# microsoft/ptgnn

Hardware: NVIDIA H100
Metric: edges/sec per GNN layer (higher is better)
Workload: dtype f32

## Files before the change

### include/ptgnn_b200.h

```cpp
#ifndef PTGNN_B200_H_
#define PTGNN_B200_H_

#include <stddef.h>
#include <stdint.h>

#ifdef __cplusplus
extern "C" {
#endif

#define PTGNN_B200_ABI_VERSION 4
#define PTGNN_MAX_EDGE_TYPES 128

enum {
    PTGNN_OK = 0,
    PTGNN_E_INVALID = -1,
    PTGNN_E_UNSUPPORTED = -2,
    PTGNN_E_CUDA = -3,
    PTGNN_E_WORKSPACE = -4,
    PTGNN_E_INDEX = -5
};

enum { PTGNN_REDUCE_SUM = 0, PTGNN_REDUCE_MEAN = 1, PTGNN_REDUCE_MAX = 2, PTGNN_REDUCE_MIN = 3 };
enum { PTGNN_ACT_NONE = 0, PTGNN_ACT_GELU = 1, PTGNN_ACT_TANH = 2, PTGNN_ACT_RELU = 3 };

int ptgnn_b200_abi_version(void);
const char *ptgnn_b200_last_error(void);
int64_t ptgnn_b200_launch_count(void);

enum {
    PTGNN_KERNEL_PLAN = 0,
    PTGNN_KERNEL_MESSAGE = 1,
    PTGNN_KERNEL_REDUCE = 2,
    PTGNN_KERNEL_GRU = 3,
    PTGNN_KERNEL_DENSE = 4,
    PTGNN_KERNEL_PACK = 5,
    PTGNN_KERNEL_CATEGORIES = 6
};
int ptgnn_b200_kernel_timing_enable(int32_t enable);
int ptgnn_b200_kernel_timing_read(double *ms , int64_t *launches , int32_t ncat);

size_t ptgnn_b200_plan_workspace_bytes(int64_t num_nodes, int64_t num_edges);
int ptgnn_b200_plan_build(int64_t num_nodes, int64_t num_source_nodes ,
                          int32_t num_types,
                          const int64_t *const *src_ptrs ,
                          const int64_t *const *tgt_ptrs ,
                          const int64_t *counts , int32_t *row_ptr, int32_t *perm,
                          int32_t *pos, int32_t *src_sorted, uint8_t *etype_sorted, int32_t *src32, int32_t *tgt32,
                          int32_t *status, void *workspace, size_t workspace_bytes, void *stream);

int ptgnn_b200_plan_convert(int64_t num_nodes, int64_t num_source_nodes, int32_t num_types,
                            const int64_t *const *src_ptrs , const int64_t *const *tgt_ptrs ,
                            const int64_t *counts , int32_t *row_ptr, int32_t *src32, int32_t *tgt32, int32_t *status,
                            void *workspace, size_t workspace_bytes, void *stream);
int ptgnn_b200_plan_sort(int64_t num_nodes, int32_t num_types, const int64_t *counts , int32_t *perm, int32_t *pos,
                         int32_t *src_sorted, uint8_t *etype_sorted, const int32_t *src32, const int32_t *tgt32,
                         void *workspace, size_t workspace_bytes, void *stream);

int ptgnn_b200_segment_reduce_f32(const float *messages, const int32_t *row_ptr, const int32_t *perm,
                                  int64_t num_nodes, int64_t num_edges, int32_t dim, int32_t reduce, float *out,
                                  int64_t *arg_out, void *stream);

size_t ptgnn_b200_scatter_workspace_bytes(int64_t num_nodes, int64_t num_edges);
int ptgnn_b200_scatter_f32(const float *src, const int64_t *index, int64_t num_edges, int32_t dim, int64_t num_nodes,
                           int32_t reduce, float *out, int64_t *arg_out, int32_t *status, void *workspace,
                           size_t workspace_bytes, void *stream);

size_t ptgnn_b200_gated_workspace_bytes(int32_t bf16_states, int64_t num_nodes, int64_t num_edges, int32_t num_types,
                                        int32_t state_dim, int32_t message_dim);
size_t ptgnn_b200_gated_weight_cache_bytes(int32_t bf16_states, int32_t num_types, int32_t state_dim, int32_t message_dim);
int ptgnn_b200_gated_forward(int32_t bf16_states, const void *node_states, const void *gather_states ,
                             int64_t num_nodes, int32_t state_dim, int32_t message_dim, int32_t num_types,
                             const int64_t *type_off , const int32_t *row_ptr, const int32_t *pos, const int32_t *src32,
                             const float *const *edge_weights , const float *gru_w_ih, const float *gru_w_hh,
                             const float *gru_b_ih, const float *gru_b_hh, int32_t reduce, void *out_states, void *workspace,
                             size_t workspace_bytes, void *weight_cache, size_t weight_cache_bytes, int32_t cache_valid,
                             void *stream);

size_t ptgnn_b200_mlp_workspace_bytes(int32_t bf16_states, int64_t num_nodes, int64_t num_edges, int32_t num_types, int32_t in_dim,
                                      int32_t message_dim, int32_t out_dim, int32_t use_target_state);
int ptgnn_b200_mlp_forward(int32_t bf16_states, const void *node_states, const void *gather_states ,
                           int64_t num_nodes, int32_t in_dim, int32_t message_dim, int32_t out_dim, int32_t num_types,
                           const int64_t *type_off , const int32_t *row_ptr, const int32_t *pos, const int32_t *src32,
                           const int32_t *tgt32, const float *const *edge_weights ,
                           int32_t use_target_state, int32_t reduce, int32_t message_activation, const float *ln_weight,
                           const float *ln_bias, float ln_eps, const float *dense_weight, const float *dense_bias,
                           int32_t dense_activation, void *out_states, void *workspace, size_t workspace_bytes, void *stream);

typedef struct {
    int32_t block_targets;
    const int32_t *group_off;
    const int32_t *src_f;
    const uint8_t *tl_f;
    int32_t *status;
} ptgnn_b200_block_plan;

int32_t ptgnn_b200_block_plan_block_targets(int64_t num_nodes);
size_t ptgnn_b200_block_plan_workspace_bytes(int64_t num_nodes, int64_t num_edges, int32_t num_types, int32_t block_targets);
int ptgnn_b200_block_plan_build(int64_t num_nodes, int32_t num_types, const int64_t *type_off ,
                                const int32_t *src32, const int32_t *tgt32, int32_t block_targets, int32_t *group_off,
                                int32_t *src_f, uint8_t *tl_f, void *workspace, size_t workspace_bytes, void *stream);

int32_t ptgnn_b200_fused_supported(int32_t bf16_states, int32_t state_dim, int32_t message_dim);

size_t ptgnn_b200_gated_fused_workspace_bytes(int32_t bf16_states, int64_t num_nodes, int64_t num_source_nodes,
                                              int32_t num_types, int32_t state_dim, int32_t message_dim);
size_t ptgnn_b200_gated_fused_weight_cache_bytes(int32_t bf16_states, int32_t num_types, int32_t state_dim, int32_t message_dim);
size_t ptgnn_b200_packed_state_bytes(int64_t num_nodes, int32_t state_dim);
int ptgnn_b200_gated_forward_fused(int32_t bf16_states, const void *node_states, const void *gather_states ,
                                   const void *packed_states_in , int64_t num_nodes,
                                   int64_t num_source_nodes, int32_t state_dim, int32_t message_dim, int32_t num_types,
                                   const ptgnn_b200_block_plan *block_plan, const int32_t *row_ptr,
                                   const float *const *edge_weights , const float *gru_w_ih,
                                   const float *gru_w_hh, const float *gru_b_ih, const float *gru_b_hh, int32_t reduce,
                                   void *out_states, void *packed_states_out , void *workspace,
                                   size_t workspace_bytes, void *weight_cache, size_t weight_cache_bytes, int32_t cache_valid,
                                   void *stream);

size_t ptgnn_b200_mlp_fused_workspace_bytes(int32_t bf16_states, int64_t num_nodes, int64_t num_source_nodes, int32_t num_types,
                                            int32_t in_dim, int32_t message_dim, int32_t out_dim, int32_t use_target_state);
size_t ptgnn_b200_mlp_fused_weight_cache_bytes(int32_t bf16_states, int32_t num_types, int32_t in_dim, int32_t message_dim, int32_t out_dim,
                                               int32_t use_target_state);
int ptgnn_b200_mlp_forward_fused(int32_t bf16_states, const void *node_states, const void *gather_states ,
                                 int64_t num_nodes, int64_t num_source_nodes, int32_t in_dim, int32_t message_dim,
                                 int32_t out_dim, int32_t num_types, const ptgnn_b200_block_plan *block_plan,
                                 const int32_t *row_ptr, const float *const *edge_weights ,
                                 int32_t use_target_state, int32_t reduce, int32_t message_activation, const float *ln_weight,
                                 const float *ln_bias, float ln_eps, const float *dense_weight, const float *dense_bias,
                                 int32_t dense_activation, void *out_states, void *workspace, size_t workspace_bytes,
                                 void *weight_cache, size_t weight_cache_bytes, int32_t cache_valid, void *stream);

int ptgnn_b200_gather_split_f16(const float *x, const int32_t *index, int64_t rows_out, int32_t cols, const float *scale, void *hi,
                                void *lo, void *stream);
int ptgnn_b200_gru_gate_grads_f32(const float *gi, const float *gh, const float *h, const float *grad_out, int64_t num_nodes,
                                  int32_t state_dim, float *d_gi, float *d_gh, float *d_h_direct, void *stream);

int ptgnn_b200_offset_ids(const int32_t *local_ids, int64_t num_items, const int64_t *item_ptr, const int64_t *node_ptr,
                          int32_t num_graphs, int64_t *out, void *stream);
int ptgnn_b200_segment_ids(const int64_t *item_ptr, int32_t num_segments, int64_t num_items, int64_t *out, void *stream);

size_t ptgnn_b200_linear_workspace_bytes(int32_t in_dim, int32_t out_dim);
int ptgnn_b200_linear_f32(const float *x, int64_t rows, int32_t in_dim, const float *weight ,
                          const float *bias , int32_t out_dim, int32_t activation, float *out, void *workspace,
                          size_t workspace_bytes, void *stream);
size_t ptgnn_b200_grucell_workspace_bytes(int32_t state_dim, int32_t input_dim);
int ptgnn_b200_grucell_f32(const float *input, const float *hidden, int64_t rows, int32_t state_dim, int32_t input_dim,
                           const float *w_ih, const float *w_hh, const float *b_ih, const float *b_hh, float *out, void *workspace,
                           size_t workspace_bytes, void *stream);
size_t ptgnn_b200_edge_messages_workspace_bytes(int32_t num_types, int32_t in_dim, int32_t message_dim, int32_t use_target_state);
int ptgnn_b200_edge_messages_f32(const float *source_states, const float *target_states ,
                                 int32_t in_dim, int32_t message_dim, int32_t num_types, const int64_t *type_off ,
                                 const int32_t *src32, const int32_t *tgt32, const int32_t *out_row,
                                 const float *const *edge_weights , int32_t use_target_state,
                                 float *messages, void *workspace, size_t workspace_bytes, void *stream);

enum { PTGNN_READOUT_SUM = 0, PTGNN_READOUT_MEAN = 1, PTGNN_READOUT_WEIGHTED_SUM = 2 };
size_t ptgnn_b200_graph_readout_workspace_bytes(int64_t num_nodes, int64_t num_graphs, int32_t state_dim);
int ptgnn_b200_graph_readout(int32_t bf16_states, const void *node_states, int64_t num_nodes, int32_t state_dim, const int32_t *row_ptr,
                             const int32_t *perm, int64_t num_graphs, const float *gate_weight ,
                             int32_t mode, float *g, float *s , void *workspace, size_t workspace_bytes, void *stream);
int32_t ptgnn_b200_global_gru_supported(int32_t bf16_states, int32_t state_dim);
size_t ptgnn_b200_global_gru_workspace_bytes(int32_t bf16_states, int64_t num_nodes, int64_t num_graphs, int32_t state_dim,
                                             int32_t summary_dim);
size_t ptgnn_b200_global_gru_weight_cache_bytes(int32_t bf16_states, int32_t state_dim);
int ptgnn_b200_global_gru_update(int32_t bf16_states, const void *node_states, const void *packed_states_in, int64_t num_nodes,
                                 int32_t state_dim, const int32_t *graph_of_node, int64_t num_graphs, const float *g, int32_t summary_dim,
                                 const float *gru_w_ih, const float *gru_w_hh, const float *gru_b_ih, const float *gru_b_hh,
                                 void *out_states, void *packed_states_out, int32_t *status, void *workspace, size_t workspace_bytes,
                                 void *weight_cache, size_t weight_cache_bytes, int32_t cache_valid, void *stream);

int32_t ptgnn_b200_attention_readout_supported(int32_t bf16_states, int32_t state_dim, int32_t num_heads);
size_t ptgnn_b200_attention_readout_workspace_bytes(int64_t num_nodes, int64_t num_graphs, int32_t state_dim, int32_t num_heads);
int ptgnn_b200_attention_readout(int32_t bf16_states, const void *node_states, int64_t num_nodes, int32_t state_dim, int32_t num_heads,
                                 const int32_t *row_ptr, const int32_t *perm, int64_t num_graphs, const float *qt, float *o, float *lse,
                                 void *workspace, size_t workspace_bytes, void *stream);
int ptgnn_b200_attention_readout_backward_f32(const float *node_states, int64_t num_nodes, int32_t state_dim, int32_t num_heads,
                                              const int32_t *row_ptr, const int32_t *perm, int64_t num_graphs, const float *qt,
                                              const float *o, const float *lse, const float *d_o, float *d_x, float *d_qt,
                                              void *workspace, size_t workspace_bytes, void *stream);

int32_t ptgnn_b200_selfatt_supported(int32_t bf16_states, int32_t key_query_dim, int32_t value_dim);
size_t ptgnn_b200_selfatt_workspace_bytes(int64_t rows, int64_t num_graphs, int32_t num_heads);
int ptgnn_b200_selfatt_forward(int32_t bf16_states, const void *qkv, int64_t rows, int32_t num_heads, int32_t key_query_dim,
                               int32_t value_dim, const int32_t *row_ptr, int64_t num_graphs, int64_t max_chunk, void *o, float *lse,
                               int32_t *status, void *workspace, size_t workspace_bytes, void *stream);
int ptgnn_b200_selfatt_backward_f32(const float *qkv, int64_t rows, int32_t num_heads, int32_t key_query_dim, int32_t value_dim,
                                    const int32_t *row_ptr, int64_t num_graphs, int64_t max_chunk, const float *o, const float *lse,
                                    const float *d_o, float *d_qkv, void *workspace, size_t workspace_bytes, void *stream);

int32_t ptgnn_b200_graph_norm_supported(int32_t state_dim);
size_t ptgnn_b200_graph_norm_workspace_bytes(int64_t num_nodes, int64_t num_graphs, int32_t state_dim);
int ptgnn_b200_graph_norm_forward(int32_t bf16_states, const void *node_states, int64_t num_nodes, int32_t state_dim, const int32_t *row_ptr,
                                  const int32_t *perm, const int32_t *graph_of_node, int64_t num_graphs, const float *gamma,
                                  const float *alpha, const float *bias, float eps, void *out, float *mean, float *rstd, void *workspace,
                                  size_t workspace_bytes, void *stream);
int ptgnn_b200_graph_norm_backward_f32(const float *node_states, const float *d_out, int64_t num_nodes, int32_t state_dim,
                                       const int32_t *row_ptr, const int32_t *perm, const int32_t *graph_of_node, int64_t num_graphs,
                                       const float *gamma, const float *alpha, float eps, const float *mean, const float *rstd, float *d_x,
                                       float *d_gamma, float *d_alpha, float *d_bias, void *workspace, size_t workspace_bytes, void *stream);

int ptgnn_b200_gated_gnn_forward_host_f32(const float *node_states, int64_t num_nodes, int32_t state_dim,
                                          int32_t num_types, const int64_t *const *src_ptrs,
                                          const int64_t *const *tgt_ptrs, const int64_t *counts, int32_t num_layers,
                                          const float *const *edge_weights ,
                                          const float *const *gru_w_ih, const float *const *gru_w_hh,
                                          const float *const *gru_b_ih, const float *const *gru_b_hh,
                                          int32_t reduce, float *out_states);

#ifdef __cplusplus
}
#endif
#endif
```

### ptgnn_b200/_native.py

```python
import ctypes
import os
from typing import Optional, Sequence

import torch

_HERE = os.path.dirname(os.path.abspath(__file__))
LIB_PATH = os.path.join(_HERE, "libptgnn_b200.so")

REDUCE = {"sum": 0, "add": 0, "mean": 1, "max": 2, "min": 3}
READOUT_SUM, READOUT_MEAN, READOUT_WEIGHTED_SUM = 0, 1, 2
ACT_NONE, ACT_GELU, ACT_TANH, ACT_RELU = 0, 1, 2, 3

c_i32, c_i64, c_f32, c_void_p, c_size_t = ctypes.c_int32, ctypes.c_int64, ctypes.c_float, ctypes.c_void_p, ctypes.c_size_t

SIGNATURES = {
    "ptgnn_b200_abi_version": (ctypes.c_int, []),
    "ptgnn_b200_last_error": (ctypes.c_char_p, []),
    "ptgnn_b200_launch_count": (c_i64, []),
    "ptgnn_b200_kernel_timing_enable": (ctypes.c_int, [c_i32]),
    "ptgnn_b200_kernel_timing_read": (ctypes.c_int, [c_void_p, c_void_p, c_i32]),
    "ptgnn_b200_plan_workspace_bytes": (c_size_t, [c_i64, c_i64]),
    "ptgnn_b200_plan_build": (ctypes.c_int, [c_i64, c_i64, c_i32, c_void_p, c_void_p, c_void_p] + [c_void_p] * 8 + [c_void_p, c_size_t, c_void_p]),
    "ptgnn_b200_plan_convert": (ctypes.c_int, [c_i64, c_i64, c_i32, c_void_p, c_void_p, c_void_p, c_void_p, c_void_p, c_void_p, c_void_p, c_void_p, c_size_t, c_void_p]),
    "ptgnn_b200_plan_sort": (ctypes.c_int, [c_i64, c_i32, c_void_p, c_void_p, c_void_p, c_void_p, c_void_p, c_void_p, c_void_p, c_void_p, c_size_t, c_void_p]),
    "ptgnn_b200_segment_reduce_f32": (ctypes.c_int, [c_void_p, c_void_p, c_void_p, c_i64, c_i64, c_i32, c_i32, c_void_p, c_void_p, c_void_p]),
    "ptgnn_b200_scatter_workspace_bytes": (c_size_t, [c_i64, c_i64]),
    "ptgnn_b200_scatter_f32": (ctypes.c_int, [c_void_p, c_void_p, c_i64, c_i32, c_i64, c_i32, c_void_p, c_void_p, c_void_p, c_void_p, c_size_t, c_void_p]),
    "ptgnn_b200_gated_workspace_bytes": (c_size_t, [c_i32, c_i64, c_i64, c_i32, c_i32, c_i32]),
    "ptgnn_b200_gated_weight_cache_bytes": (c_size_t, [c_i32, c_i32, c_i32, c_i32]),
    "ptgnn_b200_gated_forward": (ctypes.c_int, [c_i32, c_void_p, c_void_p, c_i64, c_i32, c_i32, c_i32, c_void_p, c_void_p, c_void_p, c_void_p,
                                                c_void_p, c_void_p, c_void_p, c_void_p, c_void_p, c_i32, c_void_p, c_void_p, c_size_t,
                                                c_void_p, c_size_t, c_i32, c_void_p]),
    "ptgnn_b200_mlp_workspace_bytes": (c_size_t, [c_i32, c_i64, c_i64, c_i32, c_i32, c_i32, c_i32, c_i32]),
    "ptgnn_b200_mlp_forward": (ctypes.c_int, [c_i32, c_void_p, c_void_p, c_i64, c_i32, c_i32, c_i32, c_i32, c_void_p, c_void_p, c_void_p, c_void_p,
                                              c_void_p, c_void_p, c_i32, c_i32, c_i32, c_void_p, c_void_p, c_f32, c_void_p, c_void_p, c_i32,
                                              c_void_p, c_void_p, c_size_t, c_void_p]),
    "ptgnn_b200_block_plan_block_targets": (c_i32, [c_i64]),
    "ptgnn_b200_block_plan_workspace_bytes": (c_size_t, [c_i64, c_i64, c_i32, c_i32]),
    "ptgnn_b200_block_plan_build": (ctypes.c_int, [c_i64, c_i32, c_void_p, c_void_p, c_void_p, c_i32, c_void_p, c_void_p, c_void_p, c_void_p, c_size_t, c_void_p]),
    "ptgnn_b200_fused_supported": (c_i32, [c_i32, c_i32, c_i32]),
    "ptgnn_b200_gated_fused_workspace_bytes": (c_size_t, [c_i32, c_i64, c_i64, c_i32, c_i32, c_i32]),
    "ptgnn_b200_gated_fused_weight_cache_bytes": (c_size_t, [c_i32, c_i32, c_i32, c_i32]),
    "ptgnn_b200_packed_state_bytes": (c_size_t, [c_i64, c_i32]),
    "ptgnn_b200_gated_forward_fused": (ctypes.c_int, [c_i32, c_void_p, c_void_p, c_void_p, c_i64, c_i64, c_i32, c_i32, c_i32, c_void_p, c_void_p,
                                                      c_void_p, c_void_p, c_void_p, c_void_p, c_void_p, c_i32, c_void_p, c_void_p, c_void_p,
                                                      c_size_t, c_void_p, c_size_t, c_i32, c_void_p]),
    "ptgnn_b200_mlp_fused_workspace_bytes": (c_size_t, [c_i32, c_i64, c_i64, c_i32, c_i32, c_i32, c_i32, c_i32]),
    "ptgnn_b200_mlp_fused_weight_cache_bytes": (c_size_t, [c_i32, c_i32, c_i32, c_i32, c_i32, c_i32]),
    "ptgnn_b200_mlp_forward_fused": (ctypes.c_int, [c_i32, c_void_p, c_void_p, c_i64, c_i64, c_i32, c_i32, c_i32, c_i32, c_void_p, c_void_p, c_void_p,
                                                    c_i32, c_i32, c_i32, c_void_p, c_void_p, c_f32, c_void_p, c_void_p, c_i32, c_void_p, c_void_p,
                                                    c_size_t, c_void_p, c_size_t, c_i32, c_void_p]),
    "ptgnn_b200_gather_split_f16": (ctypes.c_int, [c_void_p, c_void_p, c_i64, c_i32, c_void_p, c_void_p, c_void_p, c_void_p]),
    "ptgnn_b200_gru_gate_grads_f32": (ctypes.c_int, [c_void_p, c_void_p, c_void_p, c_void_p, c_i64, c_i32, c_void_p, c_void_p, c_void_p, c_void_p]),
    "ptgnn_b200_offset_ids": (ctypes.c_int, [c_void_p, c_i64, c_void_p, c_void_p, c_i32, c_void_p, c_void_p]),
    "ptgnn_b200_segment_ids": (ctypes.c_int, [c_void_p, c_i32, c_i64, c_void_p, c_void_p]),
    "ptgnn_b200_linear_workspace_bytes": (c_size_t, [c_i32, c_i32]),
    "ptgnn_b200_linear_f32": (ctypes.c_int, [c_void_p, c_i64, c_i32, c_void_p, c_void_p, c_i32, c_i32, c_void_p, c_void_p, c_size_t, c_void_p]),
    "ptgnn_b200_grucell_workspace_bytes": (c_size_t, [c_i32, c_i32]),
    "ptgnn_b200_grucell_f32": (ctypes.c_int, [c_void_p, c_void_p, c_i64, c_i32, c_i32, c_void_p, c_void_p, c_void_p, c_void_p, c_void_p, c_void_p, c_size_t, c_void_p]),
    "ptgnn_b200_edge_messages_workspace_bytes": (c_size_t, [c_i32, c_i32, c_i32, c_i32]),
    "ptgnn_b200_edge_messages_f32": (ctypes.c_int, [c_void_p, c_void_p, c_i32, c_i32, c_i32, c_void_p, c_void_p, c_void_p, c_void_p, c_void_p,
                                                    c_i32, c_void_p, c_void_p, c_size_t, c_void_p]),
    "ptgnn_b200_graph_readout_workspace_bytes": (c_size_t, [c_i64, c_i64, c_i32]),
    "ptgnn_b200_graph_readout": (ctypes.c_int, [c_i32, c_void_p, c_i64, c_i32, c_void_p, c_void_p, c_i64, c_void_p, c_i32, c_void_p, c_void_p,
                                                c_void_p, c_size_t, c_void_p]),
    "ptgnn_b200_global_gru_supported": (c_i32, [c_i32, c_i32]),
    "ptgnn_b200_global_gru_workspace_bytes": (c_size_t, [c_i32, c_i64, c_i64, c_i32, c_i32]),
    "ptgnn_b200_global_gru_weight_cache_bytes": (c_size_t, [c_i32, c_i32]),
    "ptgnn_b200_global_gru_update": (ctypes.c_int, [c_i32, c_void_p, c_void_p, c_i64, c_i32, c_void_p, c_i64, c_void_p, c_i32, c_void_p, c_void_p,
                                                    c_void_p, c_void_p, c_void_p, c_void_p, c_void_p, c_void_p, c_size_t, c_void_p, c_size_t,
                                                    c_i32, c_void_p]),
    "ptgnn_b200_attention_readout_supported": (c_i32, [c_i32, c_i32, c_i32]),
    "ptgnn_b200_attention_readout_workspace_bytes": (c_size_t, [c_i64, c_i64, c_i32, c_i32]),
    "ptgnn_b200_attention_readout": (ctypes.c_int, [c_i32, c_void_p, c_i64, c_i32, c_i32, c_void_p, c_void_p, c_i64, c_void_p, c_void_p,
                                                    c_void_p, c_void_p, c_size_t, c_void_p]),
    "ptgnn_b200_attention_readout_backward_f32": (ctypes.c_int, [c_void_p, c_i64, c_i32, c_i32, c_void_p, c_void_p, c_i64, c_void_p, c_void_p,
                                                                 c_void_p, c_void_p, c_void_p, c_void_p, c_void_p, c_size_t, c_void_p]),
    "ptgnn_b200_selfatt_supported": (c_i32, [c_i32, c_i32, c_i32]),
    "ptgnn_b200_selfatt_workspace_bytes": (c_size_t, [c_i64, c_i64, c_i32]),
    "ptgnn_b200_selfatt_forward": (ctypes.c_int, [c_i32, c_void_p, c_i64, c_i32, c_i32, c_i32, c_void_p, c_i64, c_i64, c_void_p, c_void_p,
                                                  c_void_p, c_void_p, c_size_t, c_void_p]),
    "ptgnn_b200_selfatt_backward_f32": (ctypes.c_int, [c_void_p, c_i64, c_i32, c_i32, c_i32, c_void_p, c_i64, c_i64, c_void_p, c_void_p,
                                                       c_void_p, c_void_p, c_void_p, c_size_t, c_void_p]),
    "ptgnn_b200_graph_norm_supported": (c_i32, [c_i32]),
    "ptgnn_b200_graph_norm_workspace_bytes": (c_size_t, [c_i64, c_i64, c_i32]),
    "ptgnn_b200_graph_norm_forward": (ctypes.c_int, [c_i32, c_void_p, c_i64, c_i32, c_void_p, c_void_p, c_void_p, c_i64, c_void_p, c_void_p,
                                                     c_void_p, c_f32, c_void_p, c_void_p, c_void_p, c_void_p, c_size_t, c_void_p]),
    "ptgnn_b200_graph_norm_backward_f32": (ctypes.c_int, [c_void_p, c_void_p, c_i64, c_i32, c_void_p, c_void_p, c_void_p, c_i64, c_void_p,
                                                          c_void_p, c_f32, c_void_p, c_void_p, c_void_p, c_void_p, c_void_p, c_void_p,
                                                          c_void_p, c_size_t, c_void_p]),
    "ptgnn_b200_gated_gnn_forward_host_f32":(ctypes.c_int, [c_void_p, c_i64, c_i32, c_i32, c_void_p, c_void_p, c_void_p, c_i32,
                                                             c_void_p, c_void_p, c_void_p, c_void_p, c_void_p, c_i32, c_void_p]),
}



class BlockPlanStruct(ctypes.Structure):
    _fields_ = [("block_targets", c_i32), ("group_off", c_void_p), ("src_f", c_void_p), ("tl_f", c_void_p), ("status", c_void_p)]


ABI_VERSION = 4
_lib: Optional[ctypes.CDLL] = None


class NativeLibraryError(RuntimeError):
    pass


def lib() -> ctypes.CDLL:
    global _lib
    if _lib is None:
        if not os.path.exists(LIB_PATH):
            raise NativeLibraryError(
                f"{LIB_PATH} not found: build it with `python -m ptgnn_b200.build` (or __graft_entry__.build()). "
                "ptgnn_b200 has no CPU / PyTorch fallback for its CUDA kernels."
            )
        handle = ctypes.CDLL(LIB_PATH)
        for name, (res, args) in SIGNATURES.items():
            fn = getattr(handle, name)
            fn.restype = res
            fn.argtypes = args
        if handle.ptgnn_b200_abi_version() != ABI_VERSION:
            raise NativeLibraryError("libptgnn_b200.so ABI version mismatch; rebuild")
        _lib = handle
    return _lib


def check(rc: int, what: str) -> None:
    if rc != 0:
        msg = lib().ptgnn_b200_last_error().decode("utf-8", "replace")
        codes = {-1: ValueError, -2: NotImplementedError, -3: RuntimeError, -4: RuntimeError, -5: IndexError}
        raise codes.get(rc, RuntimeError)(f"{what} failed (code {rc}): {msg}")


def launch_count() -> int:
    return int(lib().ptgnn_b200_launch_count())


KERNEL_CATEGORIES = ("plan", "message", "reduce", "gru", "dense", "pack")


def kernel_timing(enable: bool) -> None:
    check(lib().ptgnn_b200_kernel_timing_enable(int(enable)), "kernel_timing_enable")


def read_kernel_timing() -> dict:
    n = len(KERNEL_CATEGORIES)
    ms = (ctypes.c_double * n)()
    cnt = (c_i64 * n)()
    check(lib().ptgnn_b200_kernel_timing_read(ms, cnt, n), "kernel_timing_read")
    return {name: (float(ms[i]), int(cnt[i])) for i, name in enumerate(KERNEL_CATEGORIES)}


def ptr(t: Optional[torch.Tensor]) -> Optional[int]:
    return None if t is None else t.data_ptr()


def ptr_table(tensors: Sequence[torch.Tensor]):
    tab = (c_void_p * max(len(tensors), 1))()
    for i, t in enumerate(tensors):
        tab[i] = t.data_ptr()
    return tab


def i64_array(values: Sequence[int]):
    arr = (c_i64 * max(len(values), 1))()
    for i, v in enumerate(values):
        arr[i] = int(v)
    return arr


def current_stream(device: torch.device) -> int:
    return torch.cuda.current_stream(device).cuda_stream


def require_cuda(t: torch.Tensor, name: str, dtype: torch.dtype) -> torch.Tensor:
    if not t.is_cuda:
        raise NativeLibraryError(
            f"{name} is on {t.device}; ptgnn_b200 only runs on CUDA (sm_90a) and has no CPU fallback"
        )
    if t.dtype != dtype:
        raise TypeError(f"{name} must be {dtype}, got {t.dtype}")
    return t if t.is_contiguous() else t.contiguous()
```

### ptgnn_b200/csrc/plan.cu

```cuda
#include "common.cuh"

namespace ptgnn {

constexpr int SCAN_THREADS = 256;
constexpr int SCAN_ITEMS = 16;
constexpr int SCAN_CHUNK = SCAN_THREADS * SCAN_ITEMS;

__device__ __forceinline__ int warp_inclusive_scan(int v) {
    const int lane = threadIdx.x & 31;
#pragma unroll
    for (int o = 1; o < 32; o <<= 1) {
        int n = __shfl_up_sync(0xffffffffu, v, o);
        if (lane >= o) v += n;
    }
    return v;
}

template <int THREADS>
__device__ __forceinline__ int block_exclusive_scan(int v, int *total) {
    __shared__ int warp_sums[THREADS / 32];
    __shared__ int block_total;
    const int lane = threadIdx.x & 31, warp = threadIdx.x >> 5;
    int incl = warp_inclusive_scan(v);
    if (lane == 31) warp_sums[warp] = incl;
    __syncthreads();
    if (warp == 0) {
        int s = lane < THREADS / 32 ? warp_sums[lane] : 0;
        int si = warp_inclusive_scan(s);
        if (lane < THREADS / 32) warp_sums[lane] = si - s;
        if (lane == THREADS / 32 - 1) block_total = si;
    }
    __syncthreads();
    int res = incl - v + warp_sums[warp];
    *total = block_total;
    __syncthreads();
    return res;
}

__global__ void __launch_bounds__(SCAN_THREADS) scan_block_sums_kernel(const int32_t *__restrict__ in, int64_t n,
                                                                       int32_t *__restrict__ sums) {
    const int64_t base = (int64_t)blockIdx.x * SCAN_CHUNK + (int64_t)threadIdx.x * SCAN_ITEMS;
    int s = 0;
#pragma unroll
    for (int i = 0; i < SCAN_ITEMS; ++i)
        if (base + i < n) s += in[base + i];
    int total;
    block_exclusive_scan<SCAN_THREADS>(s, &total);
    if (threadIdx.x == 0) sums[blockIdx.x] = total;
}

__global__ void __launch_bounds__(1024) scan_sums_kernel(int32_t *__restrict__ sums, int64_t nb) {
    int carry = 0;
    for (int64_t base = 0; base < nb; base += 1024) {
        int64_t i = base + threadIdx.x;
        int v = i < nb ? sums[i] : 0;
        int total;
        int ex = block_exclusive_scan<1024>(v, &total);
        if (i < nb) sums[i] = ex + carry;
        carry += total;
    }
}

__global__ void __launch_bounds__(SCAN_THREADS) scan_apply_kernel(const int32_t *in , int64_t n,
                                                                  const int32_t *__restrict__ sums, int32_t *out,
                                                                  int32_t *out_total) {
    const int64_t base = (int64_t)blockIdx.x * SCAN_CHUNK + (int64_t)threadIdx.x * SCAN_ITEMS;
    int v[SCAN_ITEMS];
    int s = 0;
#pragma unroll
    for (int i = 0; i < SCAN_ITEMS; ++i) {
        v[i] = base + i < n ? in[base + i] : 0;
        s += v[i];
    }
    int total;
    int ex = block_exclusive_scan<SCAN_THREADS>(s, &total) + sums[blockIdx.x];
#pragma unroll
    for (int i = 0; i < SCAN_ITEMS; ++i) {
        if (base + i < n) out[base + i] = ex;
        ex += v[i];
    }
    if (out_total != nullptr && blockIdx.x == gridDim.x - 1 && threadIdx.x == SCAN_THREADS - 1) out_total[0] = ex;
}

static size_t scan_workspace_elems(int64_t n) { return (size_t)ceil_div(n > 0 ? n : 1, SCAN_CHUNK) + 1; }

static int exclusive_scan_i32(const int32_t *in, int32_t *out, int64_t n, int32_t *sums, int32_t *out_total,
                              cudaStream_t st) {
    if (n <= 0) return PTGNN_OK;
    const int64_t nb = ceil_div(n, SCAN_CHUNK);
    {
        TimedScope timed__(PTGNN_KERNEL_PLAN, st);
        scan_block_sums_kernel<<<(unsigned)nb, SCAN_THREADS, 0, st>>>(in, n, sums);
    }
    PTGNN_LAUNCHED();
    {
        TimedScope timed__(PTGNN_KERNEL_PLAN, st);
        scan_sums_kernel<<<1, 1024, 0, st>>>(sums, nb);
    }
    PTGNN_LAUNCHED();
    {
        TimedScope timed__(PTGNN_KERNEL_PLAN, st);
        scan_apply_kernel<<<(unsigned)nb, SCAN_THREADS, 0, st>>>(in, n, sums, out, out_total);
    }
    PTGNN_LAUNCHED();
    return PTGNN_OK;
}

__global__ void __launch_bounds__(256) convert_count_kernel(const __grid_constant__ EdgeTables tabs, int64_t num_nodes,
                                                            int64_t num_source_nodes, int64_t num_edges, int32_t *__restrict__ src32,
                                                            int32_t *__restrict__ tgt32, int32_t *__restrict__ deg,
                                                            int32_t *__restrict__ status) {
    int bad = 0;
    for (int64_t e = (int64_t)blockIdx.x * blockDim.x + threadIdx.x; e < num_edges;
         e += (int64_t)gridDim.x * blockDim.x) {
        const int t = type_of_edge(tabs.off, tabs.num_types, e);
        const int64_t i = e - tabs.off[t];
        int64_t s = tabs.src[t][i], v = tabs.tgt[t][i];
        if (s < 0 || s >= num_source_nodes) { s = 0; ++bad; }
        if (v < 0 || v >= num_nodes) { v = 0; ++bad; }
        src32[e] = (int32_t)s;
        tgt32[e] = (int32_t)v;
        atomicAdd(&deg[v], 1);
    }
    if (bad) atomicAdd(status, bad);
}

constexpr int RADIX_BITS = 8;
constexpr int RADIX = 1 << RADIX_BITS;
constexpr int SORT_THREADS = 256;
constexpr int SORT_WARPS = SORT_THREADS / 32;
constexpr int SORT_ROUNDS = 8;
constexpr int SORT_CHUNK = SORT_THREADS * SORT_ROUNDS;

__global__ void __launch_bounds__(SORT_THREADS) radix_hist_kernel(const int32_t *__restrict__ keys, int64_t n, int shift,
                                                                  int32_t *__restrict__ hist ) {
    __shared__ int h[RADIX];
    h[threadIdx.x] = 0;
    __syncthreads();
    const int64_t base = (int64_t)blockIdx.x * SORT_CHUNK;
#pragma unroll
    for (int r = 0; r < SORT_ROUNDS; ++r) {
        int64_t i = base + r * SORT_THREADS + threadIdx.x;
        if (i < n) atomicAdd(&h[(keys[i] >> shift) & (RADIX - 1)], 1);
    }
    __syncthreads();
    hist[(int64_t)threadIdx.x * gridDim.x + blockIdx.x] = h[threadIdx.x];
}

__global__ void __launch_bounds__(SORT_THREADS) radix_scatter_kernel(const int32_t *__restrict__ keys_in,
                                                                     const int32_t *__restrict__ vals_in, int64_t n,
                                                                     int shift, int first_pass,
                                                                     const int32_t *__restrict__ hist_scanned,
                                                                     int32_t *__restrict__ keys_out,
                                                                     int32_t *__restrict__ vals_out) {
    __shared__ int warp_hist[SORT_WARPS][RADIX];
    const int lane = threadIdx.x & 31, warp = threadIdx.x >> 5;
    for (int i = threadIdx.x; i < SORT_WARPS * RADIX; i += SORT_THREADS) (&warp_hist[0][0])[i] = 0;
    __syncthreads();

    const int64_t base = (int64_t)blockIdx.x * SORT_CHUNK + warp * (32 * SORT_ROUNDS);
    int32_t key[SORT_ROUNDS], val[SORT_ROUNDS];
    int digit[SORT_ROUNDS];
#pragma unroll
    for (int r = 0; r < SORT_ROUNDS; ++r) {
        const int64_t i = base + r * 32 + lane;
        const bool valid = i < n;
        key[r] = valid ? keys_in[i] : 0;
        val[r] = valid ? (first_pass ? (int32_t)i : vals_in[i]) : 0;
        digit[r] = valid ? ((key[r] >> shift) & (RADIX - 1)) : RADIX;
        const unsigned peers = __match_any_sync(0xffffffffu, digit[r]);
        if (valid && lane == __ffs(peers) - 1) warp_hist[warp][digit[r]] += __popc(peers);
        __syncwarp();
    }
    __syncthreads();
    {
        int run = hist_scanned[(int64_t)threadIdx.x * gridDim.x + blockIdx.x];
#pragma unroll
        for (int w = 0; w < SORT_WARPS; ++w) {
            int c = warp_hist[w][threadIdx.x];
            warp_hist[w][threadIdx.x] = run;
            run += c;
        }
    }
    __syncthreads();
#pragma unroll
    for (int r = 0; r < SORT_ROUNDS; ++r) {
        const bool valid = digit[r] < RADIX;
        const unsigned peers = __match_any_sync(0xffffffffu, digit[r]);
        int dst = 0;
        if (valid) dst = warp_hist[warp][digit[r]] + __popc(peers & ((1u << lane) - 1u));
        __syncwarp();
        if (valid && lane == __ffs(peers) - 1) warp_hist[warp][digit[r]] += __popc(peers);
        __syncwarp();
        if (valid) {
            keys_out[dst] = key[r];
            vals_out[dst] = val[r];
        }
    }
}

__global__ void __launch_bounds__(256) finalize_plan_kernel(const __grid_constant__ TypeOffsets toff, int64_t num_edges,
                                                            const int32_t *__restrict__ perm,
                                                            const int32_t *__restrict__ src32,
                                                            int32_t *__restrict__ pos, int32_t *__restrict__ src_sorted,
                                                            uint8_t *__restrict__ etype_sorted) {
    for (int64_t j = (int64_t)blockIdx.x * blockDim.x + threadIdx.x; j < num_edges;
         j += (int64_t)gridDim.x * blockDim.x) {
        const int32_t e = perm[j];
        pos[e] = (int32_t)j;
        src_sorted[j] = src32[e];
        etype_sorted[j] = (uint8_t)type_of_edge(toff.off, toff.num_types, e);
    }
}

struct PlanWs {
    size_t deg, scan_sums, keys_a, keys_b, vals_a, vals_b, hist, hist_sums, total;
};
static PlanWs plan_ws_layout(int64_t N, int64_t E) {
    PlanWs w{};
    const int64_t nblk = ceil_div(E > 0 ? E : 1, SORT_CHUNK);
    size_t o = 0;
    auto add = [&](size_t cnt) { size_t at = o; o += ws_slice(cnt, 4); return at; };
    w.deg = add((size_t)N + 1);
    w.scan_sums = add(scan_workspace_elems(N + 1));
    w.keys_a = add((size_t)E + 1);
    w.keys_b = add((size_t)E + 1);
    w.vals_a = add((size_t)E + 1);
    w.vals_b = add((size_t)E + 1);
    w.hist = add((size_t)RADIX * nblk);
    w.hist_sums = add(scan_workspace_elems((int64_t)RADIX * nblk));
    w.total = o;
    return w;
}

static int sort_edges_by_key(const int32_t *keys_in, int key_bits, int64_t E, int32_t *perm, char *ws, const PlanWs &L,
                             cudaStream_t st, const int32_t **sorted_keys = nullptr) {
    const int64_t nblk = ceil_div(E, SORT_CHUNK);
    int32_t *keys[2] = {reinterpret_cast<int32_t *>(ws + L.keys_a), reinterpret_cast<int32_t *>(ws + L.keys_b)};
    int32_t *vals[2] = {reinterpret_cast<int32_t *>(ws + L.vals_a), reinterpret_cast<int32_t *>(ws + L.vals_b)};
    int32_t *hist = reinterpret_cast<int32_t *>(ws + L.hist);
    int32_t *hist_sums = reinterpret_cast<int32_t *>(ws + L.hist_sums);
    const int passes = (key_bits + RADIX_BITS - 1) / RADIX_BITS;
    const int32_t *kin = keys_in;
    const int32_t *vin = nullptr;
    for (int p = 0; p < passes; ++p) {
        int32_t *kout = keys[p & 1];
        int32_t *vout = (p == passes - 1) ? perm : vals[p & 1];
        {
            TimedScope timed__(PTGNN_KERNEL_PLAN, st);
            radix_hist_kernel<<<(unsigned)nblk, SORT_THREADS, 0, st>>>(kin, E, p * RADIX_BITS, hist);
        }
        PTGNN_LAUNCHED();
        int rc = exclusive_scan_i32(hist, hist, (int64_t)RADIX * nblk, hist_sums, nullptr, st);
        if (rc) return rc;
        {
            TimedScope timed__(PTGNN_KERNEL_PLAN, st);
            radix_scatter_kernel<<<(unsigned)nblk, SORT_THREADS, 0, st>>>(kin, vin, E, p * RADIX_BITS, p == 0, hist, kout,
                                                                      vout);
        }
        PTGNN_LAUNCHED();
        kin = kout;
        vin = vout;
    }
    if (sorted_keys) *sorted_keys = kin;
    return PTGNN_OK;
}
static int bits_for(int64_t n) {
    int bits = 1;
    while (bits < 31 && ((int64_t)1 << bits) < n) ++bits;
    return bits;
}
static int sort_edges_by_target(const int32_t *tgt32, int64_t N, int64_t E, int32_t *perm, char *ws, const PlanWs &L,
                                cudaStream_t st) {
    return sort_edges_by_key(tgt32, bits_for(N), E, perm, ws, L, st);
}

__global__ void __launch_bounds__(256) block_keys_kernel(const __grid_constant__ TypeOffsets toff, int64_t num_edges,
                                                         const int32_t *__restrict__ tgt32, int B, int32_t *__restrict__ keys,
                                                         int32_t *__restrict__ group_count) {
    for (int64_t e = (int64_t)blockIdx.x * blockDim.x + threadIdx.x; e < num_edges; e += (int64_t)gridDim.x * blockDim.x) {
        const int t = type_of_edge(toff.off, toff.num_types, e);
        const int v = tgt32[e];
        const int blk = v / B, tl = v - blk * B;
        keys[e] = (blk * toff.num_types + t) * B + tl;
        atomicAdd(&group_count[(int64_t)blk * toff.num_types + t], 1);
    }
}
__global__ void __launch_bounds__(256) block_finalize_kernel(int64_t num_edges, int B, const int32_t *__restrict__ perm,
                                                             const int32_t *__restrict__ sorted_keys,
                                                             const int32_t *__restrict__ src32, int32_t *__restrict__ src_f,
                                                             uint8_t *__restrict__ tl_f) {
    for (int64_t j = (int64_t)blockIdx.x * blockDim.x + threadIdx.x; j < num_edges; j += (int64_t)gridDim.x * blockDim.x) {
        src_f[j] = src32[perm[j]];
        tl_f[j] = (uint8_t)(sorted_keys[j] % B);
    }
}
struct BlockPlanWs { size_t keys, perm, scan_sums, plan, total; };
static BlockPlanWs block_plan_ws_layout(int64_t N, int64_t E, int T, int B) {
    BlockPlanWs w{};
    const int64_t nblk = ceil_div(N > 0 ? N : 1, B), groups = nblk * (T > 0 ? T : 1) + 1;
    size_t o = 0;
    auto add = [&](size_t cnt) { size_t at = o; o += ws_slice(cnt, 4); return at; };
    w.keys = add((size_t)E + 1);
    w.perm = add((size_t)E + 1);
    w.scan_sums = add(scan_workspace_elems(groups));
    w.plan = o; o += plan_ws_layout(N, E).total;
    w.total = o;
    return w;
}

}

using namespace ptgnn;

extern "C" size_t ptgnn_b200_plan_workspace_bytes(int64_t num_nodes, int64_t num_edges) {
    if (num_nodes < 0 || num_edges < 0) return 0;
    return plan_ws_layout(num_nodes, num_edges).total;
}

static int plan_build_phases(int phases, int64_t num_nodes, int64_t num_source_nodes, int32_t num_types,
                             const int64_t *const *src_ptrs, const int64_t *const *tgt_ptrs, const int64_t *counts, int32_t *row_ptr,
                             int32_t *perm, int32_t *pos, int32_t *src_sorted, uint8_t *etype_sorted, int32_t *src32, int32_t *tgt32,
                             int32_t *status, void *workspace, size_t workspace_bytes, void *stream) {
    cudaStream_t st = static_cast<cudaStream_t>(stream);
    PTGNN_CHECK_ARG(num_nodes >= 0 && num_nodes < INT32_MAX, "plan_build: num_nodes=%lld out of range", (long long)num_nodes);
    if (num_source_nodes <= 0) num_source_nodes = num_nodes;
    PTGNN_CHECK_ARG(num_source_nodes < INT32_MAX, "plan_build: num_source_nodes out of range");
    PTGNN_CHECK_ARG(num_types >= 0 && num_types <= PTGNN_MAX_EDGE_TYPES, "plan_build: num_types=%d (max %d)", num_types,
                    PTGNN_MAX_EDGE_TYPES);
    PTGNN_CHECK_ARG(row_ptr && status, "plan_build: null row_ptr/status");
    EdgeTables tabs{};
    TypeOffsets toff{};
    tabs.num_types = toff.num_types = num_types;
    int64_t E = 0;
    for (int t = 0; t < num_types; ++t) {
        PTGNN_CHECK_ARG(counts[t] >= 0, "plan_build: negative edge count for type %d", t);
        PTGNN_CHECK_ARG(counts[t] == 0 || !(phases & 1) || (src_ptrs[t] && tgt_ptrs[t]), "plan_build: null edge list for type %d", t);
        tabs.src[t] = (phases & 1) ? src_ptrs[t] : nullptr;
        tabs.tgt[t] = (phases & 1) ? tgt_ptrs[t] : nullptr;
        tabs.off[t] = E;
        toff.off[t] = (int32_t)E;
        E += counts[t];
        PTGNN_CHECK_ARG(E < INT32_MAX, "plan_build: more than 2^31-1 edges");
    }
    tabs.off[num_types] = E;
    toff.off[num_types] = (int32_t)E;
    for (int t = num_types + 1; t <= PTGNN_MAX_EDGE_TYPES; ++t) { tabs.off[t] = E; toff.off[t] = (int32_t)E; }

    const PlanWs L = plan_ws_layout(num_nodes, E);
    if (workspace_bytes < L.total || (L.total && !workspace)) {
        set_error("plan_build: workspace %zu < required %zu", workspace_bytes, L.total);
        return PTGNN_E_WORKSPACE;
    }
    char *ws = static_cast<char *>(workspace);
    int32_t *deg = reinterpret_cast<int32_t *>(ws + L.deg);

    const unsigned grid = (unsigned)(ceil_div(E > 0 ? E : 1, 256) < 132 * 16 ? ceil_div(E > 0 ? E : 1, 256) : 132 * 16);
    int rc = PTGNN_OK;
    if (phases & 1) {
        PTGNN_CUDA(cudaMemsetAsync(status, 0, sizeof(int32_t), st));
        PTGNN_CUDA(cudaMemsetAsync(deg, 0, sizeof(int32_t) * (size_t)(num_nodes + 1), st));
        if (E == 0) {
            PTGNN_CUDA(cudaMemsetAsync(row_ptr, 0, sizeof(int32_t) * (size_t)(num_nodes + 1), st));
            return PTGNN_OK;
        }
        PTGNN_CHECK_ARG(src32 && tgt32, "plan_build: null output array");
        PTGNN_CHECK_ARG(num_nodes > 0, "plan_build: edges given but num_nodes == 0");
        {
            TimedScope timed__(PTGNN_KERNEL_PLAN, st);
            convert_count_kernel<<<grid, 256, 0, st>>>(tabs, num_nodes, num_source_nodes, E, src32, tgt32, deg, status);
        }
        PTGNN_LAUNCHED();
        rc = exclusive_scan_i32(deg, row_ptr, num_nodes + 1, reinterpret_cast<int32_t *>(ws + L.scan_sums), nullptr, st);
        if (rc) return rc;
    }
    if (!(phases & 2) || E == 0) return PTGNN_OK;
    PTGNN_CHECK_ARG(perm && pos && src_sorted && etype_sorted && src32 && tgt32, "plan_build: null output array");
    rc = sort_edges_by_target(tgt32, num_nodes, E, perm, ws, L, st);
    if (rc) return rc;
    {
        TimedScope timed__(PTGNN_KERNEL_PLAN, st);
        finalize_plan_kernel<<<grid, 256, 0, st>>>(toff, E, perm, src32, pos, src_sorted, etype_sorted);
    }
    PTGNN_LAUNCHED();
    return PTGNN_OK;
}

extern "C" int ptgnn_b200_plan_build(int64_t num_nodes, int64_t num_source_nodes, int32_t num_types,
                                     const int64_t *const *src_ptrs, const int64_t *const *tgt_ptrs, const int64_t *counts,
                                     int32_t *row_ptr, int32_t *perm, int32_t *pos, int32_t *src_sorted, uint8_t *etype_sorted,
                                     int32_t *src32, int32_t *tgt32, int32_t *status, void *workspace, size_t workspace_bytes,
                                     void *stream) {
    return plan_build_phases(3, num_nodes, num_source_nodes, num_types, src_ptrs, tgt_ptrs, counts, row_ptr, perm, pos, src_sorted,
                             etype_sorted, src32, tgt32, status, workspace, workspace_bytes, stream);
}
extern "C" int ptgnn_b200_plan_convert(int64_t num_nodes, int64_t num_source_nodes, int32_t num_types,
                                       const int64_t *const *src_ptrs, const int64_t *const *tgt_ptrs, const int64_t *counts,
                                       int32_t *row_ptr, int32_t *src32, int32_t *tgt32, int32_t *status, void *workspace,
                                       size_t workspace_bytes, void *stream) {
    return plan_build_phases(1, num_nodes, num_source_nodes, num_types, src_ptrs, tgt_ptrs, counts, row_ptr, nullptr, nullptr, nullptr,
                             nullptr, src32, tgt32, status, workspace, workspace_bytes, stream);
}
extern "C" int ptgnn_b200_plan_sort(int64_t num_nodes, int32_t num_types, const int64_t *counts, int32_t *perm, int32_t *pos,
                                    int32_t *src_sorted, uint8_t *etype_sorted, const int32_t *src32, const int32_t *tgt32,
                                    void *workspace, size_t workspace_bytes, void *stream) {
    int32_t dummy_status = 0;
    return plan_build_phases(2, num_nodes, num_nodes, num_types, nullptr, nullptr, counts, &dummy_status , perm, pos,
                             src_sorted, etype_sorted, const_cast<int32_t *>(src32), const_cast<int32_t *>(tgt32), &dummy_status, workspace,
                             workspace_bytes, stream);
}

extern "C" size_t ptgnn_b200_block_plan_workspace_bytes(int64_t num_nodes, int64_t num_edges, int32_t num_types,
                                                        int32_t block_targets) {
    if (num_nodes < 0 || num_edges < 0 || num_types < 0 || block_targets <= 0) return 0;
    return block_plan_ws_layout(num_nodes, num_edges, num_types, block_targets).total;
}

extern "C" int ptgnn_b200_block_plan_build(int64_t num_nodes, int32_t num_types, const int64_t *type_off,
                                           const int32_t *src32, const int32_t *tgt32, int32_t block_targets,
                                           int32_t *group_off, int32_t *src_f, uint8_t *tl_f, void *workspace,
                                           size_t workspace_bytes, void *stream) {
    cudaStream_t st = static_cast<cudaStream_t>(stream);
    const int B = block_targets, T = num_types;
    PTGNN_CHECK_ARG(num_nodes >= 0 && num_nodes < INT32_MAX, "block_plan_build: num_nodes out of range");
    PTGNN_CHECK_ARG(T > 0 && T <= PTGNN_MAX_EDGE_TYPES && type_off, "block_plan_build: bad num_types=%d", T);
    PTGNN_CHECK_ARG(B >= 8 && B <= 256, "block_plan_build: block_targets=%d must be in [8, 256]", B);
    const int64_t E = type_off[T];
    PTGNN_CHECK_ARG(E >= 0 && E < INT32_MAX, "block_plan_build: edge count out of range");
    const int64_t nblk = ceil_div(num_nodes, B), groups = nblk * T;
    PTGNN_CHECK_ARG(nblk * T * B < ((int64_t)1 << 31), "block_plan_build: %lld blocks x %d types x %d targets overflow the 31-bit sort key",
                    (long long)nblk, T, B);
    PTGNN_CHECK_ARG(group_off, "block_plan_build: null group_off");
    const BlockPlanWs L = block_plan_ws_layout(num_nodes, E, T, B);
    if (workspace_bytes < L.total || !workspace) {
        set_error("block_plan_build: workspace %zu < required %zu", workspace_bytes, L.total);
        return PTGNN_E_WORKSPACE;
    }
    PTGNN_CUDA(cudaMemsetAsync(group_off, 0, sizeof(int32_t) * (size_t)(groups + 1), st));
    if (E == 0 || num_nodes == 0) return PTGNN_OK;
    PTGNN_CHECK_ARG(src32 && tgt32 && src_f && tl_f, "block_plan_build: null edge array");
    char *ws = static_cast<char *>(workspace);
    int32_t *keys = reinterpret_cast<int32_t *>(ws + L.keys), *perm = reinterpret_cast<int32_t *>(ws + L.perm);
    TypeOffsets toff{};
    toff.num_types = T;
    for (int t = 0; t <= PTGNN_MAX_EDGE_TYPES; ++t) toff.off[t] = (int32_t)type_off[t < T ? t : T];
    const unsigned grid = (unsigned)(ceil_div(E, 256) < 132 * 16 ? ceil_div(E, 256) : 132 * 16);
    {
        TimedScope timed__(PTGNN_KERNEL_PLAN, st);
        block_keys_kernel<<<grid, 256, 0, st>>>(toff, E, tgt32, B, keys, group_off);
    }
    PTGNN_LAUNCHED();
    int rc = exclusive_scan_i32(group_off, group_off, groups + 1, reinterpret_cast<int32_t *>(ws + L.scan_sums), nullptr, st);
    if (rc) return rc;
    const int32_t *sorted_keys = nullptr;
    rc = sort_edges_by_key(keys, bits_for(nblk * T * B), E, perm, ws + L.plan, plan_ws_layout(num_nodes, E), st, &sorted_keys);
    if (rc) return rc;
    {
        TimedScope timed__(PTGNN_KERNEL_PLAN, st);
        block_finalize_kernel<<<grid, 256, 0, st>>>(E, B, perm, sorted_keys, src32, src_f, tl_f);
    }
    PTGNN_LAUNCHED();
    return PTGNN_OK;
}
```

### ptgnn_b200/edgeplan.py

```python
import os
import threading
from collections import OrderedDict
from typing import List, Optional, Sequence, Tuple

import torch

from . import _native as N

Adjacency = Sequence[Tuple[torch.Tensor, torch.Tensor]]


class EdgePlan:

    __slots__ = (
        "num_nodes", "num_source_nodes", "num_edges", "num_types", "type_off", "type_off_c", "row_ptr", "src32", "tgt32", "status", "device", "_keepalive", "_validated", "_block", "_sorted", "_counts_c",
        "_block_targets",
    )

    STATUS_WORDS = 4

    def __init__(self, adjacency_lists: Adjacency, num_nodes: int, validate: bool = False,
                 num_source_nodes: Optional[int] = None, block_targets: Optional[int] = None):
        if block_targets is not None:
            bt = int(block_targets)
            if bt != block_targets or bt % 8 != 0 or not 8 <= bt <= 176:
                raise ValueError(f"block_targets={block_targets!r} must be a multiple of 8 in [8, 176]")
            block_targets = bt
        self._block_targets = block_targets
        if len(adjacency_lists) > 128:
            raise NotImplementedError("more than 128 edge types")
        if len(adjacency_lists) == 0:
            raise ValueError("at least one edge type is required")
        device = adjacency_lists[0][0].device
        srcs = [N.require_cuda(s, f"adjacency_lists[{i}][0]", torch.int64) for i, (s, _) in enumerate(adjacency_lists)]
        tgts = [N.require_cuda(t, f"adjacency_lists[{i}][1]", torch.int64) for i, (_, t) in enumerate(adjacency_lists)]
        counts = [int(s.shape[0]) for s in srcs]
        for s, t in zip(srcs, tgts):
            if s.dim() != 1 or t.shape != s.shape:
                raise ValueError("adjacency lists must be pairs of equal-length 1-D tensors")
        E = sum(counts)
        self.num_nodes, self.num_edges, self.num_types, self.device = int(num_nodes), E, len(counts), device
        self.num_source_nodes = int(num_source_nodes) if num_source_nodes is not None else int(num_nodes)
        self.type_off = [0]
        for c in counts:
            self.type_off.append(self.type_off[-1] + c)
        self.type_off_c = N.i64_array(self.type_off)

        def i32(n):
            return torch.empty(n, dtype=torch.int32, device=device)

        self.row_ptr = i32(num_nodes + 1)
        self.src32, self.tgt32 = i32(E), i32(E)
        self._sorted = None
        self.status = torch.zeros(self.STATUS_WORDS, dtype=torch.int32).pin_memory()
        self._block = None
        self._counts_c = N.i64_array(counts)
        lib = N.lib()
        ws_bytes = lib.ptgnn_b200_plan_workspace_bytes(num_nodes, E)
        ws = torch.empty(max(ws_bytes, 1), dtype=torch.uint8, device=device)
        with torch.cuda.device(device):
            rc = lib.ptgnn_b200_plan_convert(
                num_nodes, self.num_source_nodes, len(counts), N.ptr_table(srcs), N.ptr_table(tgts), self._counts_c,
                N.ptr(self.row_ptr), N.ptr(self.src32), N.ptr(self.tgt32), N.ptr(self.status), N.ptr(ws), ws_bytes,
                N.current_stream(device),
            )
        N.check(rc, "ptgnn_b200_plan_convert")
        self._keepalive = (srcs, tgts)
        self._validated = False
        if validate:
            self.validate()

    def _sort(self):
        if self._sorted is None:
            E, dev = self.num_edges, self.device
            perm, pos, src_sorted = (torch.empty(E, dtype=torch.int32, device=dev) for _ in range(3))
            etype_sorted = torch.empty(E, dtype=torch.uint8, device=dev)
            if E:
                lib = N.lib()
                ws_bytes = lib.ptgnn_b200_plan_workspace_bytes(self.num_nodes, E)
                ws = torch.empty(max(ws_bytes, 1), dtype=torch.uint8, device=dev)
                with torch.cuda.device(dev):
                    rc = lib.ptgnn_b200_plan_sort(self.num_nodes, self.num_types, self._counts_c, N.ptr(perm), N.ptr(pos), N.ptr(src_sorted),
                                                  N.ptr(etype_sorted), N.ptr(self.src32), N.ptr(self.tgt32), N.ptr(ws), ws_bytes,
                                                  N.current_stream(dev))
                N.check(rc, "ptgnn_b200_plan_sort")
            self._sorted = (perm, pos, src_sorted, etype_sorted)
        return self._sorted

    perm = property(lambda self: self._sort()[0])
    pos = property(lambda self: self._sort()[1])
    src_sorted = property(lambda self: self._sort()[2])
    etype_sorted = property(lambda self: self._sort()[3])

    def validate(self) -> None:
        if not self._validated:
            torch.cuda.current_stream(self.device).synchronize()
            self.poll()
            self._validated = True

    def poll(self) -> None:
        st = self.status
        if int(st[0]):
            raise IndexError(f"{int(st[0])} edge indices outside [0, {self.num_nodes}) (targets) / [0, {self.num_source_nodes}) "
                             "(sources); the kernels route such edges to node 0, results are not valid")
        if int(st[1]) or int(st[2]):
            what = "node states" if int(st[1]) else "edge weights"
            raise FloatingPointError(
                f"{what} outside the fp16 range (|x| >= 65504, inf or NaN) reached the fp32-exact fused kernel (3xFP16 split); "
                "set PTGNN_B200_FP32_MODE=tf32 to use the unfused 3xTF32 kernels for such inputs")

    def block_plan(self) -> "N.BlockPlanStruct":
        if self._block is None:
            lib = N.lib()
            B = self._block_targets
            if B is None:
                B = int(lib.ptgnn_b200_block_plan_block_targets(self.num_nodes))
            nblk = (self.num_nodes + B - 1) // B
            dev = self.device
            group_off = torch.empty(nblk * self.num_types + 1, dtype=torch.int32, device=dev)
            src_f = torch.empty(max(self.num_edges, 1), dtype=torch.int32, device=dev)
            tl_f = torch.empty(max(self.num_edges, 1), dtype=torch.uint8, device=dev)
            ws_bytes = lib.ptgnn_b200_block_plan_workspace_bytes(self.num_nodes, self.num_edges, self.num_types, B)
            ws = torch.empty(max(ws_bytes, 1), dtype=torch.uint8, device=dev)
            with torch.cuda.device(dev):
                rc = lib.ptgnn_b200_block_plan_build(self.num_nodes, self.num_types, self.type_off_c, N.ptr(self.src32), N.ptr(self.tgt32),
                                                     B, N.ptr(group_off), N.ptr(src_f), N.ptr(tl_f), N.ptr(ws), ws_bytes,
                                                     N.current_stream(dev))
            N.check(rc, "ptgnn_b200_block_plan_build")
            struct = N.BlockPlanStruct(B, N.ptr(group_off), N.ptr(src_f), N.ptr(tl_f), self.status.data_ptr() + 4)
            self._block = (struct, group_off, src_f, tl_f, B)
        return self._block[0]

    @property
    def block_targets(self) -> int:
        self.block_plan()
        return self._block[4]


_CACHE: "OrderedDict[tuple, EdgePlan]" = OrderedDict()
_CACHE_SIZE = 4


def _version(t: torch.Tensor):
    try:
        return t._version
    except RuntimeError:
        return object()


def _key(adjacency_lists: Adjacency, num_nodes: int, num_source_nodes: Optional[int] = None) -> tuple:
    parts: list = [num_nodes, -1 if num_source_nodes is None else num_source_nodes]
    for s, t in adjacency_lists:
        parts += [s.data_ptr(), s.shape[0], _version(s), t.data_ptr(), _version(t)]
    return tuple(parts)


_TLS = threading.local()


def current_shared_plan() -> Optional[EdgePlan]:
    return getattr(_TLS, "plan", None)


class shared_plan:

    def __init__(self, plan: Optional[EdgePlan]):
        self.plan, self.previous = plan, None

    def __enter__(self):
        self.previous = getattr(_TLS, "plan", None)
        _TLS.plan = self.plan
        return self.plan

    def __exit__(self, *exc):
        _TLS.plan = self.previous
        return False


class shared_num_graphs:

    def __init__(self, num_graphs: Optional[int]):
        self.num_graphs, self.previous = num_graphs, None

    def __enter__(self):
        self.previous = getattr(_TLS, "num_graphs", None)
        _TLS.num_graphs = self.num_graphs
        return self.num_graphs

    def __exit__(self, *exc):
        _TLS.num_graphs = self.previous
        return False


def current_num_graphs() -> Optional[int]:
    return getattr(_TLS, "num_graphs", None)


class state_chain:

    def __init__(self):
        self.want_output = False
        self._tensor: Optional[torch.Tensor] = None
        self._packed: Optional[torch.Tensor] = None
        self._version = None
        self.previous = None

    def __enter__(self):
        self.previous = getattr(_TLS, "chain", None)
        _TLS.chain = self
        return self

    def __exit__(self, *exc):
        _TLS.chain = self.previous
        self._tensor = self._packed = None
        return False

    def lookup(self, node_states: torch.Tensor) -> Optional[torch.Tensor]:
        if self._tensor is node_states and self._packed is not None and _version(node_states) == self._version:
            return self._packed
        return None

    def store(self, out_states: torch.Tensor, packed: Optional[torch.Tensor]) -> None:
        self._tensor, self._packed = (out_states, packed) if packed is not None else (None, None)
        self._version = _version(out_states) if packed is not None else None


def current_state_chain() -> Optional[state_chain]:
    if os.environ.get("PTGNN_B200_CHAIN", "1") == "0":
        return None
    return getattr(_TLS, "chain", None)


def plan_for(adjacency_lists: Adjacency, num_nodes: int, plan: Optional[EdgePlan] = None,
             num_source_nodes: Optional[int] = None) -> EdgePlan:
    if plan is not None and _matches(plan, adjacency_lists, num_nodes, num_source_nodes):
        plan.poll()
        return plan
    key = _key(adjacency_lists, num_nodes, num_source_nodes)
    hit = _CACHE.get(key)
    if hit is not None:
        _CACHE.move_to_end(key)
        hit.poll()
        return hit
    built = EdgePlan(adjacency_lists, num_nodes, num_source_nodes=num_source_nodes)
    _CACHE[key] = built
    while len(_CACHE) > _CACHE_SIZE:
        _CACHE.popitem(last=False)
    return built


def _matches(plan: EdgePlan, adjacency_lists: Adjacency, num_nodes: int, num_source_nodes: Optional[int]) -> bool:
    if plan.num_nodes != num_nodes or plan.num_types != len(adjacency_lists):
        return False
    if num_source_nodes is not None and plan.num_source_nodes != num_source_nodes:
        return False
    return all(plan.type_off[i + 1] - plan.type_off[i] == int(s.shape[0]) for i, (s, _) in enumerate(adjacency_lists))


def clear_plan_cache() -> None:
    _CACHE.clear()
```

Measured before the change: 1.214 billion.

## Fuse edge conversion with block plan build and use decoupled-lookback scan

Replaces the three-kernel exclusive scan with a single decoupled-lookback scan kernel that handles several segments per launch. Switches the radix sort to 11-bit digits with larger tiles and a first pass that fuses edge conversion, degree counting, block-key generation and histogramming. Adds a combined plan_convert_block entry point, and EdgePlan now builds lazily so convert and block plan run in one pipeline. The aim is fewer launches and fewer passes over the edge arrays during plan construction. The cost is more complex code that depends on inter-block spin-waiting and on larger shared-memory histograms.

```diff
diff --git a/include/ptgnn_b200.h b/include/ptgnn_b200.h
--- a/include/ptgnn_b200.h
+++ b/include/ptgnn_b200.h
@@ -99,6 +99,13 @@
 int ptgnn_b200_block_plan_build(int64_t num_nodes, int32_t num_types, const int64_t *type_off ,
                                 const int32_t *src32, const int32_t *tgt32, int32_t block_targets, int32_t *group_off,
                                 int32_t *src_f, uint8_t *tl_f, void *workspace, size_t workspace_bytes, void *stream);
+
+size_t ptgnn_b200_plan_convert_block_workspace_bytes(int64_t num_nodes, int64_t num_edges, int32_t num_types, int32_t block_targets);
+int ptgnn_b200_plan_convert_block(int64_t num_nodes, int64_t num_source_nodes , int32_t num_types,
+                                  const int64_t *const *src_ptrs , const int64_t *const *tgt_ptrs ,
+                                  const int64_t *counts , int32_t block_targets, int32_t *row_ptr, int32_t *src32,
+                                  int32_t *tgt32, int32_t *status, int32_t *group_off, int32_t *src_f, uint8_t *tl_f, void *workspace,
+                                  size_t workspace_bytes, void *stream);
 
 int32_t ptgnn_b200_fused_supported(int32_t bf16_states, int32_t state_dim, int32_t message_dim);
 
diff --git a/ptgnn_b200/_native.py b/ptgnn_b200/_native.py
--- a/ptgnn_b200/_native.py
+++ b/ptgnn_b200/_native.py
@@ -38,6 +38,9 @@
     "ptgnn_b200_block_plan_block_targets": (c_i32, [c_i64]),
     "ptgnn_b200_block_plan_workspace_bytes": (c_size_t, [c_i64, c_i64, c_i32, c_i32]),
     "ptgnn_b200_block_plan_build": (ctypes.c_int, [c_i64, c_i32, c_void_p, c_void_p, c_void_p, c_i32, c_void_p, c_void_p, c_void_p, c_void_p, c_size_t, c_void_p]),
+    "ptgnn_b200_plan_convert_block_workspace_bytes": (c_size_t, [c_i64, c_i64, c_i32, c_i32]),
+    "ptgnn_b200_plan_convert_block": (ctypes.c_int, [c_i64, c_i64, c_i32, c_void_p, c_void_p, c_void_p, c_i32] + [c_void_p] * 7
+                                      + [c_void_p, c_size_t, c_void_p]),
     "ptgnn_b200_fused_supported": (c_i32, [c_i32, c_i32, c_i32]),
     "ptgnn_b200_gated_fused_workspace_bytes": (c_size_t, [c_i32, c_i64, c_i64, c_i32, c_i32, c_i32]),
     "ptgnn_b200_gated_fused_weight_cache_bytes": (c_size_t, [c_i32, c_i32, c_i32, c_i32]),
diff --git a/ptgnn_b200/csrc/plan.cu b/ptgnn_b200/csrc/plan.cu
--- a/ptgnn_b200/csrc/plan.cu
+++ b/ptgnn_b200/csrc/plan.cu
@@ -1,10 +1,6 @@
 #include "common.cuh"
 
 namespace ptgnn {
-
-constexpr int SCAN_THREADS = 256;
-constexpr int SCAN_ITEMS = 16;
-constexpr int SCAN_CHUNK = SCAN_THREADS * SCAN_ITEMS;
 
 __device__ __forceinline__ int warp_inclusive_scan(int v) {
     const int lane = threadIdx.x & 31;
@@ -37,34 +33,49 @@
     return res;
 }
 
-__global__ void __launch_bounds__(SCAN_THREADS) scan_block_sums_kernel(const int32_t *__restrict__ in, int64_t n,
-                                                                       int32_t *__restrict__ sums) {
-    const int64_t base = (int64_t)blockIdx.x * SCAN_CHUNK + (int64_t)threadIdx.x * SCAN_ITEMS;
-    int s = 0;
-#pragma unroll
-    for (int i = 0; i < SCAN_ITEMS; ++i)
-        if (base + i < n) s += in[base + i];
-    int total;
-    block_exclusive_scan<SCAN_THREADS>(s, &total);
-    if (threadIdx.x == 0) sums[blockIdx.x] = total;
-}
-
-__global__ void __launch_bounds__(1024) scan_sums_kernel(int32_t *__restrict__ sums, int64_t nb) {
-    int carry = 0;
-    for (int64_t base = 0; base < nb; base += 1024) {
-        int64_t i = base + threadIdx.x;
-        int v = i < nb ? sums[i] : 0;
-        int total;
-        int ex = block_exclusive_scan<1024>(v, &total);
-        if (i < nb) sums[i] = ex + carry;
-        carry += total;
-    }
-}
-
-__global__ void __launch_bounds__(SCAN_THREADS) scan_apply_kernel(const int32_t *in , int64_t n,
-                                                                  const int32_t *__restrict__ sums, int32_t *out,
-                                                                  int32_t *out_total) {
-    const int64_t base = (int64_t)blockIdx.x * SCAN_CHUNK + (int64_t)threadIdx.x * SCAN_ITEMS;
+constexpr int SCAN_THREADS = 256;
+constexpr int SCAN_ITEMS = 16;
+constexpr int SCAN_TILE = SCAN_THREADS * SCAN_ITEMS;
+constexpr int SCAN_MAX_SEGS = 3;
+constexpr unsigned long long FLAG_AGGREGATE = 1ull << 32, FLAG_INCLUSIVE = 2ull << 32;
+
+struct ScanSeg {
+    const int32_t *in;
+    int32_t *out;
+    int64_t n;
+    int32_t first_tile;
+};
+struct ScanJob {
+    ScanSeg seg[SCAN_MAX_SEGS];
+    int num_segs;
+    int32_t *tile_counter;
+    unsigned long long *flags;
+    const int32_t *status_in;
+    int32_t *status_out;
+};
+
+__device__ __forceinline__ unsigned long long ld_relaxed_u64(const unsigned long long *p) {
+    unsigned long long v;
+    asm volatile("ld.relaxed.gpu.global.u64 %0, [%1];" : "=l"(v) : "l"(p) : "memory");
+    return v;
+}
+__device__ __forceinline__ void st_relaxed_u64(unsigned long long *p, unsigned long long v) {
+    asm volatile("st.relaxed.gpu.global.u64 [%0], %1;" ::"l"(p), "l"(v) : "memory");
+}
+
+__global__ void __launch_bounds__(SCAN_THREADS) scan_segments_kernel(const __grid_constant__ ScanJob job) {
+    __shared__ int s_tile, s_prefix;
+    if (threadIdx.x == 0) s_tile = atomicAdd(job.tile_counter, 1);
+    __syncthreads();
+    const int tile = s_tile;
+    int k = 0;
+    while (k + 1 < job.num_segs && tile >= job.seg[k + 1].first_tile) ++k;
+    const int32_t *in = job.seg[k].in;
+    int32_t *out = job.seg[k].out;
+    const int64_t n = job.seg[k].n;
+    const int first = job.seg[k].first_tile;
+
+    const int64_t base = (int64_t)(tile - first) * SCAN_TILE + (int64_t)threadIdx.x * SCAN_ITEMS;
     int v[SCAN_ITEMS];
     int s = 0;
 #pragma unroll
@@ -73,317 +84,437 @@
         s += v[i];
     }
     int total;
-    int ex = block_exclusive_scan<SCAN_THREADS>(s, &total) + sums[blockIdx.x];
+    int ex = block_exclusive_scan<SCAN_THREADS>(s, &total);
+    if (threadIdx.x < 32) {
+        const int lane = threadIdx.x;
+        int prefix = 0;
+        if (tile == first) {
+            if (lane == 0) st_relaxed_u64(&job.flags[tile], FLAG_INCLUSIVE | (uint32_t)total);
+        } else {
+            if (lane == 0) st_relaxed_u64(&job.flags[tile], FLAG_AGGREGATE | (uint32_t)total);
+            for (int hi = tile - 1;; hi -= 32) {
+                const int j = hi - lane;
+                unsigned long long f = FLAG_INCLUSIVE;
+                if (j >= first) {
+                    do { f = ld_relaxed_u64(&job.flags[j]); } while ((f >> 32) == 0);
+                }
+                const unsigned incl = __ballot_sync(0xffffffffu, (f >> 32) == (FLAG_INCLUSIVE >> 32));
+                const int stop = incl ? __ffs(incl) - 1 : 31;
+                int x = lane <= stop ? (int)(uint32_t)f : 0;
+#pragma unroll
+                for (int o = 16; o > 0; o >>= 1) x += __shfl_xor_sync(0xffffffffu, x, o);
+                prefix += x;
+                if (incl) break;
+            }
+            if (lane == 0) st_relaxed_u64(&job.flags[tile], FLAG_INCLUSIVE | (uint32_t)(prefix + total));
+        }
+        if (lane == 0) s_prefix = prefix;
+    }
+    __syncthreads();
+    ex += s_prefix;
 #pragma unroll
     for (int i = 0; i < SCAN_ITEMS; ++i) {
         if (base + i < n) out[base + i] = ex;
         ex += v[i];
     }
-    if (out_total != nullptr && blockIdx.x == gridDim.x - 1 && threadIdx.x == SCAN_THREADS - 1) out_total[0] = ex;
-}
-
-static size_t scan_workspace_elems(int64_t n) { return (size_t)ceil_div(n > 0 ? n : 1, SCAN_CHUNK) + 1; }
-
-static int exclusive_scan_i32(const int32_t *in, int32_t *out, int64_t n, int32_t *sums, int32_t *out_total,
-                              cudaStream_t st) {
-    if (n <= 0) return PTGNN_OK;
-    const int64_t nb = ceil_div(n, SCAN_CHUNK);
-    {
-        TimedScope timed__(PTGNN_KERNEL_PLAN, st);
-        scan_block_sums_kernel<<<(unsigned)nb, SCAN_THREADS, 0, st>>>(in, n, sums);
-    }
-    PTGNN_LAUNCHED();
-    {
-        TimedScope timed__(PTGNN_KERNEL_PLAN, st);
-        scan_sums_kernel<<<1, 1024, 0, st>>>(sums, nb);
-    }
-    PTGNN_LAUNCHED();
-    {
-        TimedScope timed__(PTGNN_KERNEL_PLAN, st);
-        scan_apply_kernel<<<(unsigned)nb, SCAN_THREADS, 0, st>>>(in, n, sums, out, out_total);
-    }
-    PTGNN_LAUNCHED();
-    return PTGNN_OK;
-}
-
-__global__ void __launch_bounds__(256) convert_count_kernel(const __grid_constant__ EdgeTables tabs, int64_t num_nodes,
-                                                            int64_t num_source_nodes, int64_t num_edges, int32_t *__restrict__ src32,
-                                                            int32_t *__restrict__ tgt32, int32_t *__restrict__ deg,
-                                                            int32_t *__restrict__ status) {
-    int bad = 0;
-    for (int64_t e = (int64_t)blockIdx.x * blockDim.x + threadIdx.x; e < num_edges;
-         e += (int64_t)gridDim.x * blockDim.x) {
-        const int t = type_of_edge(tabs.off, tabs.num_types, e);
-        const int64_t i = e - tabs.off[t];
-        int64_t s = tabs.src[t][i], v = tabs.tgt[t][i];
-        if (s < 0 || s >= num_source_nodes) { s = 0; ++bad; }
-        if (v < 0 || v >= num_nodes) { v = 0; ++bad; }
-        src32[e] = (int32_t)s;
-        tgt32[e] = (int32_t)v;
-        atomicAdd(&deg[v], 1);
-    }
-    if (bad) atomicAdd(status, bad);
-}
-
-constexpr int RADIX_BITS = 8;
+    if (tile == 0 && threadIdx.x == 0 && job.status_out != nullptr) job.status_out[0] = job.status_in[0];
+}
+
+constexpr int RADIX_BITS = 11;
 constexpr int RADIX = 1 << RADIX_BITS;
 constexpr int SORT_THREADS = 256;
 constexpr int SORT_WARPS = SORT_THREADS / 32;
-constexpr int SORT_ROUNDS = 8;
+constexpr int SORT_ROUNDS = 16;
 constexpr int SORT_CHUNK = SORT_THREADS * SORT_ROUNDS;
-
-__global__ void __launch_bounds__(SORT_THREADS) radix_hist_kernel(const int32_t *__restrict__ keys, int64_t n, int shift,
-                                                                  int32_t *__restrict__ hist ) {
-    __shared__ int h[RADIX];
-    h[threadIdx.x] = 0;
-    __syncthreads();
-    const int64_t base = (int64_t)blockIdx.x * SORT_CHUNK;
+constexpr int MAX_PASSES = 3;
+constexpr int FIRST_PASS_BATCH = 8;
+
+enum SortKey { KEY_NONE = 0, KEY_TARGET = 1, KEY_BLOCK = 2 };
+
+template <bool CONVERT, int KEY>
+__global__ void __launch_bounds__(SORT_THREADS, 3) plan_first_pass_kernel(const __grid_constant__ EdgeTables tabs, int64_t num_nodes,
+                                                                       int64_t num_source_nodes, int64_t num_edges, int32_t *__restrict__ src32,
+                                                                       int32_t *__restrict__ tgt32, int32_t *__restrict__ deg,
+                                                                       int32_t *__restrict__ bad_count, int B, int32_t *__restrict__ keys,
+                                                                       int32_t *__restrict__ group_count, int32_t *__restrict__ hist0) {
+    __shared__ int h[KEY == KEY_NONE ? 1 : RADIX];
+    if (KEY != KEY_NONE) {
+        for (int i = threadIdx.x; i < RADIX; i += SORT_THREADS) h[i] = 0;
+        __syncthreads();
+    }
+    const int lane = threadIdx.x & 31;
+    int bad = 0;
+    for (int r0 = 0; r0 < SORT_ROUNDS; r0 += FIRST_PASS_BATCH) {
+        const int64_t base = (int64_t)blockIdx.x * SORT_CHUNK + r0 * SORT_THREADS + threadIdx.x;
+        int type[FIRST_PASS_BATCH], tgt[FIRST_PASS_BATCH];
+        if (CONVERT) {
+            int64_t s64[FIRST_PASS_BATCH], v64[FIRST_PASS_BATCH];
+#pragma unroll
+            for (int r = 0; r < FIRST_PASS_BATCH; ++r) {
+                const int64_t e = base + r * SORT_THREADS;
+                type[r] = 0;
+                s64[r] = v64[r] = 0;
+                if (e < num_edges) {
+                    type[r] = type_of_edge(tabs.off, tabs.num_types, e);
+                    const int64_t i = e - tabs.off[type[r]];
+                    s64[r] = tabs.src[type[r]][i];
+                    v64[r] = tabs.tgt[type[r]][i];
+                }
+            }
+#pragma unroll
+            for (int r = 0; r < FIRST_PASS_BATCH; ++r) {
+                const int64_t e = base + r * SORT_THREADS;
+                int64_t s = s64[r], v = v64[r];
+                if (s < 0 || s >= num_source_nodes) { s = 0; ++bad; }
+                if (v < 0 || v >= num_nodes) { v = 0; ++bad; }
+                tgt[r] = (int)v;
+                if (e < num_edges) {
+                    src32[e] = (int32_t)s;
+                    tgt32[e] = (int32_t)v;
+                    atomicAdd(&deg[v], 1);
+                }
+            }
+        } else {
+#pragma unroll
+            for (int r = 0; r < FIRST_PASS_BATCH; ++r) {
+                const int64_t e = base + r * SORT_THREADS;
+                const bool valid = e < num_edges;
+                type[r] = valid && KEY == KEY_BLOCK ? type_of_edge(tabs.off, tabs.num_types, e) : 0;
+                tgt[r] = valid ? tgt32[e] : 0;
+            }
+        }
+        if (KEY != KEY_NONE) {
+#pragma unroll
+            for (int r = 0; r < FIRST_PASS_BATCH; ++r) {
+                const int64_t e = base + r * SORT_THREADS;
+                const bool valid = e < num_edges;
+                int key = tgt[r];
+                if (KEY == KEY_BLOCK) {
+                    const int blk = tgt[r] / B, tl = tgt[r] - blk * B;
+                    const int g = valid ? blk * tabs.num_types + type[r] : -1;
+                    const unsigned peers = __match_any_sync(0xffffffffu, g);
+                    if (valid && lane == __ffs(peers) - 1) atomicAdd(&group_count[g], __popc(peers));
+                    key = g * B + tl;
+                    if (valid) keys[e] = key;
+                }
+                if (valid) atomicAdd(&h[key & (RADIX - 1)], 1);
+            }
+        }
+    }
+    if (CONVERT && bad) atomicAdd(bad_count, bad);
+    if (KEY != KEY_NONE) {
+        __syncthreads();
+        for (int d = threadIdx.x; d < RADIX; d += SORT_THREADS) hist0[(int64_t)d * gridDim.x + blockIdx.x] = h[d];
+    }
+}
+
+enum ScatterMode { SCATTER_MID = 0, SCATTER_TARGET = 1, SCATTER_BLOCK = 2 };
+
+
+struct SortOutputs {
+    const int32_t *src32;
+    int32_t *perm, *pos, *src_sorted;
+    uint8_t *etype_sorted;
+    int32_t *src_f;
+    uint8_t *tl_f;
+    int B;
+    TypeOffsets toff;
+};
+
+__device__ __forceinline__ unsigned long long pack_pair(int32_t key, int32_t id) {
+    return ((unsigned long long)(uint32_t)key << 32) | (uint32_t)id;
+}
+
+template <int MODE>
+__global__ void __launch_bounds__(SORT_THREADS, 3) radix_scatter_kernel(const int32_t *__restrict__ keys_in ,
+                                                                     const unsigned long long *__restrict__ pairs_in ,
+                                                                     int64_t n, int shift, const int32_t *__restrict__ offsets,
+                                                                     unsigned long long *__restrict__ pairs_out,
+                                                                     int32_t *__restrict__ next_hist, const __grid_constant__ SortOutputs out) {
+    __shared__ uint16_t warp_hist[SORT_WARPS][RADIX];
+    __shared__ int digit_base[RADIX];
+    const int lane = threadIdx.x & 31, warp = threadIdx.x >> 5;
+    for (int i = threadIdx.x; i < SORT_WARPS * RADIX / 2; i += SORT_THREADS) reinterpret_cast<uint32_t *>(&warp_hist[0][0])[i] = 0;
+    __syncthreads();
+
+    const int64_t base = (int64_t)blockIdx.x * SORT_CHUNK + warp * (32 * SORT_ROUNDS);
+    int32_t key[SORT_ROUNDS];
+    unsigned peers[SORT_ROUNDS];
 #pragma unroll
     for (int r = 0; r < SORT_ROUNDS; ++r) {
-        int64_t i = base + r * SORT_THREADS + threadIdx.x;
-        if (i < n) atomicAdd(&h[(keys[i] >> shift) & (RADIX - 1)], 1);
-    }
-    __syncthreads();
-    hist[(int64_t)threadIdx.x * gridDim.x + blockIdx.x] = h[threadIdx.x];
-}
-
-__global__ void __launch_bounds__(SORT_THREADS) radix_scatter_kernel(const int32_t *__restrict__ keys_in,
-                                                                     const int32_t *__restrict__ vals_in, int64_t n,
-                                                                     int shift, int first_pass,
-                                                                     const int32_t *__restrict__ hist_scanned,
-                                                                     int32_t *__restrict__ keys_out,
-                                                                     int32_t *__restrict__ vals_out) {
-    __shared__ int warp_hist[SORT_WARPS][RADIX];
-    const int lane = threadIdx.x & 31, warp = threadIdx.x >> 5;
-    for (int i = threadIdx.x; i < SORT_WARPS * RADIX; i += SORT_THREADS) (&warp_hist[0][0])[i] = 0;
-    __syncthreads();
-
-    const int64_t base = (int64_t)blockIdx.x * SORT_CHUNK + warp * (32 * SORT_ROUNDS);
-    int32_t key[SORT_ROUNDS], val[SORT_ROUNDS];
-    int digit[SORT_ROUNDS];
+        const int64_t i = base + r * 32 + lane;
+        key[r] = i >= n ? 0 : pairs_in != nullptr ? (int32_t)(pairs_in[i] >> 32) : keys_in[i];
+    }
+#pragma unroll
+    for (int r = 0; r < SORT_ROUNDS; ++r) {
+        const bool valid = base + r * 32 + lane < n;
+        const int digit = valid ? ((key[r] >> shift) & (RADIX - 1)) : RADIX;
+        peers[r] = __match_any_sync(0xffffffffu, digit);
+        if (valid && lane == __ffs(peers[r]) - 1) warp_hist[warp][digit] += __popc(peers[r]);
+        __syncwarp();
+    }
+    __syncthreads();
+    for (int d = threadIdx.x; d < RADIX; d += SORT_THREADS) {
+        int run = 0;
+#pragma unroll
+        for (int w = 0; w < SORT_WARPS; ++w) {
+            const int c = warp_hist[w][d];
+            warp_hist[w][d] = (uint16_t)run;
+            run += c;
+        }
+        digit_base[d] = offsets[(int64_t)d * gridDim.x + blockIdx.x];
+    }
+    __syncthreads();
 #pragma unroll
     for (int r = 0; r < SORT_ROUNDS; ++r) {
         const int64_t i = base + r * 32 + lane;
         const bool valid = i < n;
-        key[r] = valid ? keys_in[i] : 0;
-        val[r] = valid ? (first_pass ? (int32_t)i : vals_in[i]) : 0;
-        digit[r] = valid ? ((key[r] >> shift) & (RADIX - 1)) : RADIX;
-        const unsigned peers = __match_any_sync(0xffffffffu, digit[r]);
-        if (valid && lane == __ffs(peers) - 1) warp_hist[warp][digit[r]] += __popc(peers);
+        const int digit = valid ? ((key[r] >> shift) & (RADIX - 1)) : RADIX;
+        int dst = 0;
+        if (valid) dst = digit_base[digit] + warp_hist[warp][digit] + __popc(peers[r] & ((1u << lane) - 1u));
         __syncwarp();
-    }
-    __syncthreads();
-    {
-        int run = hist_scanned[(int64_t)threadIdx.x * gridDim.x + blockIdx.x];
-#pragma unroll
-        for (int w = 0; w < SORT_WARPS; ++w) {
-            int c = warp_hist[w][threadIdx.x];
-            warp_hist[w][threadIdx.x] = run;
-            run += c;
-        }
-    }
-    __syncthreads();
-#pragma unroll
-    for (int r = 0; r < SORT_ROUNDS; ++r) {
-        const bool valid = digit[r] < RADIX;
-        const unsigned peers = __match_any_sync(0xffffffffu, digit[r]);
-        int dst = 0;
-        if (valid) dst = warp_hist[warp][digit[r]] + __popc(peers & ((1u << lane) - 1u));
-        __syncwarp();
-        if (valid && lane == __ffs(peers) - 1) warp_hist[warp][digit[r]] += __popc(peers);
+        if (valid && lane == __ffs(peers[r]) - 1) warp_hist[warp][digit] += __popc(peers[r]);
         __syncwarp();
         if (valid) {
-            keys_out[dst] = key[r];
-            vals_out[dst] = val[r];
-        }
-    }
-}
-
-__global__ void __launch_bounds__(256) finalize_plan_kernel(const __grid_constant__ TypeOffsets toff, int64_t num_edges,
-                                                            const int32_t *__restrict__ perm,
-                                                            const int32_t *__restrict__ src32,
-                                                            int32_t *__restrict__ pos, int32_t *__restrict__ src_sorted,
-                                                            uint8_t *__restrict__ etype_sorted) {
-    for (int64_t j = (int64_t)blockIdx.x * blockDim.x + threadIdx.x; j < num_edges;
-         j += (int64_t)gridDim.x * blockDim.x) {
-        const int32_t e = perm[j];
-        pos[e] = (int32_t)j;
-        src_sorted[j] = src32[e];
-        etype_sorted[j] = (uint8_t)type_of_edge(toff.off, toff.num_types, e);
-    }
-}
-
-struct PlanWs {
-    size_t deg, scan_sums, keys_a, keys_b, vals_a, vals_b, hist, hist_sums, total;
-};
-static PlanWs plan_ws_layout(int64_t N, int64_t E) {
-    PlanWs w{};
-    const int64_t nblk = ceil_div(E > 0 ? E : 1, SORT_CHUNK);
-    size_t o = 0;
-    auto add = [&](size_t cnt) { size_t at = o; o += ws_slice(cnt, 4); return at; };
-    w.deg = add((size_t)N + 1);
-    w.scan_sums = add(scan_workspace_elems(N + 1));
-    w.keys_a = add((size_t)E + 1);
-    w.keys_b = add((size_t)E + 1);
-    w.vals_a = add((size_t)E + 1);
-    w.vals_b = add((size_t)E + 1);
-    w.hist = add((size_t)RADIX * nblk);
-    w.hist_sums = add(scan_workspace_elems((int64_t)RADIX * nblk));
-    w.total = o;
-    return w;
-}
-
-static int sort_edges_by_key(const int32_t *keys_in, int key_bits, int64_t E, int32_t *perm, char *ws, const PlanWs &L,
-                             cudaStream_t st, const int32_t **sorted_keys = nullptr) {
-    const int64_t nblk = ceil_div(E, SORT_CHUNK);
-    int32_t *keys[2] = {reinterpret_cast<int32_t *>(ws + L.keys_a), reinterpret_cast<int32_t *>(ws + L.keys_b)};
-    int32_t *vals[2] = {reinterpret_cast<int32_t *>(ws + L.vals_a), reinterpret_cast<int32_t *>(ws + L.vals_b)};
-    int32_t *hist = reinterpret_cast<int32_t *>(ws + L.hist);
-    int32_t *hist_sums = reinterpret_cast<int32_t *>(ws + L.hist_sums);
-    const int passes = (key_bits + RADIX_BITS - 1) / RADIX_BITS;
-    const int32_t *kin = keys_in;
-    const int32_t *vin = nullptr;
-    for (int p = 0; p < passes; ++p) {
-        int32_t *kout = keys[p & 1];
-        int32_t *vout = (p == passes - 1) ? perm : vals[p & 1];
-        {
-            TimedScope timed__(PTGNN_KERNEL_PLAN, st);
-            radix_hist_kernel<<<(unsigned)nblk, SORT_THREADS, 0, st>>>(kin, E, p * RADIX_BITS, hist);
-        }
-        PTGNN_LAUNCHED();
-        int rc = exclusive_scan_i32(hist, hist, (int64_t)RADIX * nblk, hist_sums, nullptr, st);
-        if (rc) return rc;
-        {
-            TimedScope timed__(PTGNN_KERNEL_PLAN, st);
-            radix_scatter_kernel<<<(unsigned)nblk, SORT_THREADS, 0, st>>>(kin, vin, E, p * RADIX_BITS, p == 0, hist, kout,
-                                                                      vout);
-        }
-        PTGNN_LAUNCHED();
-        kin = kout;
-        vin = vout;
-    }
-    if (sorted_keys) *sorted_keys = kin;
-    return PTGNN_OK;
-}
+            const int32_t k = key[r], e = pairs_in != nullptr ? (int32_t)(uint32_t)pairs_in[i] : (int32_t)i;
+            if (MODE == SCATTER_MID) {
+                pairs_out[dst] = pack_pair(k, e);
+                atomicAdd(&next_hist[(int64_t)((k >> (shift + RADIX_BITS)) & (RADIX - 1)) * gridDim.x + dst / SORT_CHUNK], 1);
+            } else if (MODE == SCATTER_TARGET) {
+                out.perm[dst] = e;
+                out.pos[e] = dst;
+                out.src_sorted[dst] = out.src32[e];
+                out.etype_sorted[dst] = (uint8_t)type_of_edge(out.toff.off, out.toff.num_types, e);
+            } else {
+                out.src_f[dst] = out.src32[e];
+                out.tl_f[dst] = (uint8_t)(k % out.B);
+            }
+        }
+    }
+}
+
+constexpr int NUM_COUNTERS = 8;
+
 static int bits_for(int64_t n) {
     int bits = 1;
     while (bits < 31 && ((int64_t)1 << bits) < n) ++bits;
     return bits;
 }
-static int sort_edges_by_target(const int32_t *tgt32, int64_t N, int64_t E, int32_t *perm, char *ws, const PlanWs &L,
-                                cudaStream_t st) {
-    return sort_edges_by_key(tgt32, bits_for(N), E, perm, ws, L, st);
-}
-
-__global__ void __launch_bounds__(256) block_keys_kernel(const __grid_constant__ TypeOffsets toff, int64_t num_edges,
-                                                         const int32_t *__restrict__ tgt32, int B, int32_t *__restrict__ keys,
-                                                         int32_t *__restrict__ group_count) {
-    for (int64_t e = (int64_t)blockIdx.x * blockDim.x + threadIdx.x; e < num_edges; e += (int64_t)gridDim.x * blockDim.x) {
-        const int t = type_of_edge(toff.off, toff.num_types, e);
-        const int v = tgt32[e];
-        const int blk = v / B, tl = v - blk * B;
-        keys[e] = (blk * toff.num_types + t) * B + tl;
-        atomicAdd(&group_count[(int64_t)blk * toff.num_types + t], 1);
-    }
-}
-__global__ void __launch_bounds__(256) block_finalize_kernel(int64_t num_edges, int B, const int32_t *__restrict__ perm,
-                                                             const int32_t *__restrict__ sorted_keys,
-                                                             const int32_t *__restrict__ src32, int32_t *__restrict__ src_f,
-                                                             uint8_t *__restrict__ tl_f) {
-    for (int64_t j = (int64_t)blockIdx.x * blockDim.x + threadIdx.x; j < num_edges; j += (int64_t)gridDim.x * blockDim.x) {
-        src_f[j] = src32[perm[j]];
-        tl_f[j] = (uint8_t)(sorted_keys[j] % B);
-    }
-}
-struct BlockPlanWs { size_t keys, perm, scan_sums, plan, total; };
-static BlockPlanWs block_plan_ws_layout(int64_t N, int64_t E, int T, int B) {
-    BlockPlanWs w{};
-    const int64_t nblk = ceil_div(N > 0 ? N : 1, B), groups = nblk * (T > 0 ? T : 1) + 1;
+static int64_t scan_tiles(int64_t n) { return ceil_div(n > 0 ? n : 1, SCAN_TILE); }
+
+struct PlanWs {
+    int passes;
+    int64_t nchunks, hist_elems;
+    size_t counters, deg, gcount, flags, hist[MAX_PASSES], zero_bytes;
+    size_t keys, pairs[2], total;
+};
+static PlanWs plan_ws_layout(int64_t N, int64_t E, bool convert, int64_t groups, int key_bits) {
+    PlanWs w{};
+    w.passes = key_bits > 0 ? (key_bits + RADIX_BITS - 1) / RADIX_BITS : 0;
+    w.nchunks = ceil_div(E > 0 ? E : 1, SORT_CHUNK);
+    w.hist_elems = (int64_t)RADIX * w.nchunks;
     size_t o = 0;
-    auto add = [&](size_t cnt) { size_t at = o; o += ws_slice(cnt, 4); return at; };
-    w.keys = add((size_t)E + 1);
-    w.perm = add((size_t)E + 1);
-    w.scan_sums = add(scan_workspace_elems(groups));
-    w.plan = o; o += plan_ws_layout(N, E).total;
+    auto add = [&](int64_t cnt, size_t elt) { size_t at = o; o += ws_slice((size_t)cnt, elt); return at; };
+    w.counters = add(NUM_COUNTERS, 4);
+    w.deg = add(convert ? N + 1 : 0, 4);
+    w.gcount = add(groups > 0 ? groups + 1 : 0, 4);
+    w.flags = add((convert ? scan_tiles(N + 1) : 0) + (groups > 0 ? scan_tiles(groups + 1) : 0) + w.passes * scan_tiles(w.hist_elems), 8);
+    for (int p = 1; p < w.passes; ++p) w.hist[p] = add(w.hist_elems, 4);
+    w.zero_bytes = o;
+    if (w.passes > 0) {
+        w.hist[0] = add(w.hist_elems, 4);
+        w.keys = add(groups > 0 ? E : 0, 4);
+        for (int b = 0; b < 2; ++b) w.pairs[b] = add(E + 1, 8);
+    }
     w.total = o;
     return w;
 }
 
+struct PlanJob {
+    bool convert = false;
+    int key = KEY_NONE;
+    EdgeTables tabs{};
+    TypeOffsets toff{};
+    int64_t N = 0, N_src = 0, E = 0;
+    int T = 0, B = 0;
+    int32_t *src32 = nullptr, *tgt32 = nullptr, *row_ptr = nullptr, *status = nullptr;
+    int32_t *perm = nullptr, *pos = nullptr, *src_sorted = nullptr;
+    uint8_t *etype_sorted = nullptr;
+    int32_t *group_off = nullptr, *src_f = nullptr;
+    uint8_t *tl_f = nullptr;
+
+    int64_t groups() const { return key == KEY_BLOCK ? ceil_div(N, B) * T : 0; }
+    int key_bits() const { return key == KEY_TARGET ? bits_for(N) : key == KEY_BLOCK ? bits_for(groups() * B) : 0; }
+    PlanWs layout() const { return plan_ws_layout(N, E, convert, groups(), key_bits()); }
+};
+
+static int job_edges(PlanJob &J, int32_t num_types, const int64_t *const *src_ptrs, const int64_t *const *tgt_ptrs, const int64_t *counts,
+                     bool lists) {
+    PTGNN_CHECK_ARG(num_types >= 0 && num_types <= PTGNN_MAX_EDGE_TYPES, "plan_build: num_types=%d (max %d)", num_types,
+                    PTGNN_MAX_EDGE_TYPES);
+    J.T = J.tabs.num_types = J.toff.num_types = num_types;
+    int64_t E = 0;
+    for (int t = 0; t < num_types; ++t) {
+        PTGNN_CHECK_ARG(counts[t] >= 0, "plan_build: negative edge count for type %d", t);
+        PTGNN_CHECK_ARG(counts[t] == 0 || !lists || (src_ptrs[t] && tgt_ptrs[t]), "plan_build: null edge list for type %d", t);
+        J.tabs.src[t] = lists ? src_ptrs[t] : nullptr;
+        J.tabs.tgt[t] = lists ? tgt_ptrs[t] : nullptr;
+        J.tabs.off[t] = E;
+        J.toff.off[t] = (int32_t)E;
+        E += counts[t];
+        PTGNN_CHECK_ARG(E < INT32_MAX, "plan_build: more than 2^31-1 edges");
+    }
+    for (int t = num_types; t <= PTGNN_MAX_EDGE_TYPES; ++t) { J.tabs.off[t] = E; J.toff.off[t] = (int32_t)E; }
+    J.E = E;
+    return PTGNN_OK;
+}
+
+static int check_block_args(const PlanJob &J, const char *what) {
+    PTGNN_CHECK_ARG(J.T > 0, "%s: bad num_types=%d", what, J.T);
+    PTGNN_CHECK_ARG(J.B >= 8 && J.B <= 256, "%s: block_targets=%d must be in [8, 256]", what, J.B);
+    const int64_t nblk = ceil_div(J.N, J.B);
+    PTGNN_CHECK_ARG(nblk * J.T * J.B < ((int64_t)1 << 31), "%s: %lld blocks x %d types x %d targets overflow the 31-bit sort key", what,
+                    (long long)nblk, J.T, J.B);
+    PTGNN_CHECK_ARG(J.group_off, "%s: null group_off", what);
+    return PTGNN_OK;
+}
+
+static int64_t launch_scan(ScanJob job, int32_t *counter, unsigned long long *flags, cudaStream_t st) {
+    int64_t tiles = 0;
+    for (int k = 0; k < job.num_segs; ++k) {
+        job.seg[k].first_tile = (int32_t)tiles;
+        tiles += scan_tiles(job.seg[k].n);
+    }
+    job.tile_counter = counter;
+    job.flags = flags;
+    {
+        TimedScope timed__(PTGNN_KERNEL_PLAN, st);
+        scan_segments_kernel<<<(unsigned)tiles, SCAN_THREADS, 0, st>>>(job);
+    }
+    return tiles;
+}
+
+template <bool CONVERT, int KEY>
+static void launch_first_pass(const PlanJob &J, const PlanWs &L, char *ws, cudaStream_t st) {
+    TimedScope timed__(PTGNN_KERNEL_PLAN, st);
+    plan_first_pass_kernel<CONVERT, KEY><<<(unsigned)L.nchunks, SORT_THREADS, 0, st>>>(
+        J.tabs, J.N, J.N_src, J.E, J.src32, J.tgt32, reinterpret_cast<int32_t *>(ws + L.deg), reinterpret_cast<int32_t *>(ws + L.counters),
+        J.B, reinterpret_cast<int32_t *>(ws + L.keys), reinterpret_cast<int32_t *>(ws + L.gcount), reinterpret_cast<int32_t *>(ws + L.hist[0]));
+}
+
+static int run_plan(const PlanJob &J, void *workspace, size_t workspace_bytes, cudaStream_t st) {
+    const PlanWs L = J.layout();
+    if (workspace_bytes < L.total || (L.total && !workspace)) {
+        set_error("plan_build: workspace %zu < required %zu", workspace_bytes, L.total);
+        return PTGNN_E_WORKSPACE;
+    }
+    const int64_t groups = J.groups();
+    if (J.E == 0 || (J.key == KEY_BLOCK && J.N == 0)) {
+        if (J.convert) {
+            PTGNN_CUDA(cudaMemsetAsync(J.status, 0, sizeof(int32_t), st));
+            PTGNN_CUDA(cudaMemsetAsync(J.row_ptr, 0, sizeof(int32_t) * (size_t)(J.N + 1), st));
+        }
+        if (J.key == KEY_BLOCK) PTGNN_CUDA(cudaMemsetAsync(J.group_off, 0, sizeof(int32_t) * (size_t)(groups + 1), st));
+        return PTGNN_OK;
+    }
+    char *ws = static_cast<char *>(workspace);
+    auto i32 = [&](size_t off) { return reinterpret_cast<int32_t *>(ws + off); };
+    int32_t *counters = i32(L.counters);
+    unsigned long long *flags = reinterpret_cast<unsigned long long *>(ws + L.flags);
+    PTGNN_CUDA(cudaMemsetAsync(ws, 0, L.zero_bytes, st));
+
+    if (J.convert && J.key == KEY_NONE) launch_first_pass<true, KEY_NONE>(J, L, ws, st);
+    else if (J.convert && J.key == KEY_TARGET) launch_first_pass<true, KEY_TARGET>(J, L, ws, st);
+    else if (J.convert) launch_first_pass<true, KEY_BLOCK>(J, L, ws, st);
+    else if (J.key == KEY_TARGET) launch_first_pass<false, KEY_TARGET>(J, L, ws, st);
+    else launch_first_pass<false, KEY_BLOCK>(J, L, ws, st);
+    PTGNN_LAUNCHED();
+
+    ScanJob sj{};
+    if (J.convert) {
+        sj.seg[sj.num_segs++] = ScanSeg{i32(L.deg), J.row_ptr, J.N + 1, 0};
+        sj.status_in = counters;
+        sj.status_out = J.status;
+    }
+    if (J.key == KEY_BLOCK) sj.seg[sj.num_segs++] = ScanSeg{i32(L.gcount), J.group_off, groups + 1, 0};
+    if (J.key != KEY_NONE) sj.seg[sj.num_segs++] = ScanSeg{i32(L.hist[0]), i32(L.hist[0]), L.hist_elems, 0};
+    int scans = 0;
+    int64_t flag_off = launch_scan(sj, counters + 1 + scans++, flags, st);
+    PTGNN_LAUNCHED();
+
+    SortOutputs out{};
+    out.src32 = J.src32;
+    out.perm = J.perm;
+    out.pos = J.pos;
+    out.src_sorted = J.src_sorted;
+    out.etype_sorted = J.etype_sorted;
+    out.src_f = J.src_f;
+    out.tl_f = J.tl_f;
+    out.B = J.B;
+    out.toff = J.toff;
+    const int32_t *kin = J.key == KEY_BLOCK ? i32(L.keys) : J.tgt32;
+    const unsigned long long *pin = nullptr;
+    for (int p = 0; p < L.passes; ++p) {
+        if (p > 0) {
+            ScanJob hj{};
+            hj.seg[hj.num_segs++] = ScanSeg{i32(L.hist[p]), i32(L.hist[p]), L.hist_elems, 0};
+            flag_off += launch_scan(hj, counters + 1 + scans++, flags + flag_off, st);
+            PTGNN_LAUNCHED();
+        }
+        unsigned long long *pout = reinterpret_cast<unsigned long long *>(ws + L.pairs[p & 1]);
+        int32_t *next = p + 1 < L.passes ? i32(L.hist[p + 1]) : nullptr;
+        const int32_t *offsets = i32(L.hist[p]);
+        const unsigned grid = (unsigned)L.nchunks;
+        {
+            TimedScope timed__(PTGNN_KERNEL_PLAN, st);
+            if (p + 1 < L.passes)
+                radix_scatter_kernel<SCATTER_MID><<<grid, SORT_THREADS, 0, st>>>(kin, pin, J.E, p * RADIX_BITS, offsets, pout, next, out);
+            else if (J.key == KEY_TARGET)
+                radix_scatter_kernel<SCATTER_TARGET><<<grid, SORT_THREADS, 0, st>>>(kin, pin, J.E, p * RADIX_BITS, offsets, pout, next, out);
+            else
+                radix_scatter_kernel<SCATTER_BLOCK><<<grid, SORT_THREADS, 0, st>>>(kin, pin, J.E, p * RADIX_BITS, offsets, pout, next, out);
+        }
+        PTGNN_LAUNCHED();
+        pin = pout;
+    }
+    return PTGNN_OK;
+}
+
 }
 
 using namespace ptgnn;
 
 extern "C" size_t ptgnn_b200_plan_workspace_bytes(int64_t num_nodes, int64_t num_edges) {
     if (num_nodes < 0 || num_edges < 0) return 0;
-    return plan_ws_layout(num_nodes, num_edges).total;
+    return plan_ws_layout(num_nodes, num_edges, true, 0, bits_for(num_nodes)).total;
 }
 
 static int plan_build_phases(int phases, int64_t num_nodes, int64_t num_source_nodes, int32_t num_types,
                              const int64_t *const *src_ptrs, const int64_t *const *tgt_ptrs, const int64_t *counts, int32_t *row_ptr,
                              int32_t *perm, int32_t *pos, int32_t *src_sorted, uint8_t *etype_sorted, int32_t *src32, int32_t *tgt32,
                              int32_t *status, void *workspace, size_t workspace_bytes, void *stream) {
-    cudaStream_t st = static_cast<cudaStream_t>(stream);
     PTGNN_CHECK_ARG(num_nodes >= 0 && num_nodes < INT32_MAX, "plan_build: num_nodes=%lld out of range", (long long)num_nodes);
     if (num_source_nodes <= 0) num_source_nodes = num_nodes;
     PTGNN_CHECK_ARG(num_source_nodes < INT32_MAX, "plan_build: num_source_nodes out of range");
-    PTGNN_CHECK_ARG(num_types >= 0 && num_types <= PTGNN_MAX_EDGE_TYPES, "plan_build: num_types=%d (max %d)", num_types,
-                    PTGNN_MAX_EDGE_TYPES);
-    PTGNN_CHECK_ARG(row_ptr && status, "plan_build: null row_ptr/status");
-    EdgeTables tabs{};
-    TypeOffsets toff{};
-    tabs.num_types = toff.num_types = num_types;
-    int64_t E = 0;
-    for (int t = 0; t < num_types; ++t) {
-        PTGNN_CHECK_ARG(counts[t] >= 0, "plan_build: negative edge count for type %d", t);
-        PTGNN_CHECK_ARG(counts[t] == 0 || !(phases & 1) || (src_ptrs[t] && tgt_ptrs[t]), "plan_build: null edge list for type %d", t);
-        tabs.src[t] = (phases & 1) ? src_ptrs[t] : nullptr;
-        tabs.tgt[t] = (phases & 1) ? tgt_ptrs[t] : nullptr;
-        tabs.off[t] = E;
-        toff.off[t] = (int32_t)E;
-        E += counts[t];
-        PTGNN_CHECK_ARG(E < INT32_MAX, "plan_build: more than 2^31-1 edges");
-    }
-    tabs.off[num_types] = E;
-    toff.off[num_types] = (int32_t)E;
-    for (int t = num_types + 1; t <= PTGNN_MAX_EDGE_TYPES; ++t) { tabs.off[t] = E; toff.off[t] = (int32_t)E; }
-
-    const PlanWs L = plan_ws_layout(num_nodes, E);
-    if (workspace_bytes < L.total || (L.total && !workspace)) {
-        set_error("plan_build: workspace %zu < required %zu", workspace_bytes, L.total);
-        return PTGNN_E_WORKSPACE;
-    }
-    char *ws = static_cast<char *>(workspace);
-    int32_t *deg = reinterpret_cast<int32_t *>(ws + L.deg);
-
-    const unsigned grid = (unsigned)(ceil_div(E > 0 ? E : 1, 256) < 132 * 16 ? ceil_div(E > 0 ? E : 1, 256) : 132 * 16);
-    int rc = PTGNN_OK;
-    if (phases & 1) {
-        PTGNN_CUDA(cudaMemsetAsync(status, 0, sizeof(int32_t), st));
-        PTGNN_CUDA(cudaMemsetAsync(deg, 0, sizeof(int32_t) * (size_t)(num_nodes + 1), st));
-        if (E == 0) {
-            PTGNN_CUDA(cudaMemsetAsync(row_ptr, 0, sizeof(int32_t) * (size_t)(num_nodes + 1), st));
-            return PTGNN_OK;
-        }
-        PTGNN_CHECK_ARG(src32 && tgt32, "plan_build: null output array");
-        PTGNN_CHECK_ARG(num_nodes > 0, "plan_build: edges given but num_nodes == 0");
-        {
-            TimedScope timed__(PTGNN_KERNEL_PLAN, st);
-            convert_count_kernel<<<grid, 256, 0, st>>>(tabs, num_nodes, num_source_nodes, E, src32, tgt32, deg, status);
-        }
-        PTGNN_LAUNCHED();
-        rc = exclusive_scan_i32(deg, row_ptr, num_nodes + 1, reinterpret_cast<int32_t *>(ws + L.scan_sums), nullptr, st);
-        if (rc) return rc;
-    }
-    if (!(phases & 2) || E == 0) return PTGNN_OK;
-    PTGNN_CHECK_ARG(perm && pos && src_sorted && etype_sorted && src32 && tgt32, "plan_build: null output array");
-    rc = sort_edges_by_target(tgt32, num_nodes, E, perm, ws, L, st);
+    PlanJob J;
+    int rc = job_edges(J, num_types, src_ptrs, tgt_ptrs, counts, phases & 1);
     if (rc) return rc;
-    {
-        TimedScope timed__(PTGNN_KERNEL_PLAN, st);
-        finalize_plan_kernel<<<grid, 256, 0, st>>>(toff, E, perm, src32, pos, src_sorted, etype_sorted);
-    }
-    PTGNN_LAUNCHED();
-    return PTGNN_OK;
+    J.convert = phases & 1;
+    J.key = (phases & 2) ? KEY_TARGET : KEY_NONE;
+    J.N = num_nodes;
+    J.N_src = num_source_nodes;
+    J.src32 = src32; J.tgt32 = tgt32; J.row_ptr = row_ptr; J.status = status;
+    J.perm = perm; J.pos = pos; J.src_sorted = src_sorted; J.etype_sorted = etype_sorted;
+    if (J.convert) {
+        PTGNN_CHECK_ARG(row_ptr && status, "plan_build: null row_ptr/status");
+        if (J.E > 0) {
+            PTGNN_CHECK_ARG(src32 && tgt32, "plan_build: null output array");
+            PTGNN_CHECK_ARG(num_nodes > 0, "plan_build: edges given but num_nodes == 0");
+        }
+    }
+    if (J.key == KEY_TARGET && J.E > 0)
+        PTGNN_CHECK_ARG(perm && pos && src_sorted && etype_sorted && src32 && tgt32, "plan_build: null output array");
+    return run_plan(J, workspace, workspace_bytes, static_cast<cudaStream_t>(stream));
 }
 
 extern "C" int ptgnn_b200_plan_build(int64_t num_nodes, int64_t num_source_nodes, int32_t num_types,
@@ -404,61 +535,74 @@
 extern "C" int ptgnn_b200_plan_sort(int64_t num_nodes, int32_t num_types, const int64_t *counts, int32_t *perm, int32_t *pos,
                                     int32_t *src_sorted, uint8_t *etype_sorted, const int32_t *src32, const int32_t *tgt32,
                                     void *workspace, size_t workspace_bytes, void *stream) {
-    int32_t dummy_status = 0;
-    return plan_build_phases(2, num_nodes, num_nodes, num_types, nullptr, nullptr, counts, &dummy_status , perm, pos,
-                             src_sorted, etype_sorted, const_cast<int32_t *>(src32), const_cast<int32_t *>(tgt32), &dummy_status, workspace,
-                             workspace_bytes, stream);
+    return plan_build_phases(2, num_nodes, num_nodes, num_types, nullptr, nullptr, counts, nullptr, perm, pos, src_sorted, etype_sorted,
+                             const_cast<int32_t *>(src32), const_cast<int32_t *>(tgt32), nullptr, workspace, workspace_bytes, stream);
 }
 
 extern "C" size_t ptgnn_b200_block_plan_workspace_bytes(int64_t num_nodes, int64_t num_edges, int32_t num_types,
                                                         int32_t block_targets) {
     if (num_nodes < 0 || num_edges < 0 || num_types < 0 || block_targets <= 0) return 0;
-    return block_plan_ws_layout(num_nodes, num_edges, num_types, block_targets).total;
+    const int64_t groups = ceil_div(num_nodes, block_targets) * num_types;
+    return plan_ws_layout(num_nodes, num_edges, false, groups, bits_for(groups * block_targets)).total;
 }
 
 extern "C" int ptgnn_b200_block_plan_build(int64_t num_nodes, int32_t num_types, const int64_t *type_off,
                                            const int32_t *src32, const int32_t *tgt32, int32_t block_targets,
                                            int32_t *group_off, int32_t *src_f, uint8_t *tl_f, void *workspace,
                                            size_t workspace_bytes, void *stream) {
-    cudaStream_t st = static_cast<cudaStream_t>(stream);
-    const int B = block_targets, T = num_types;
     PTGNN_CHECK_ARG(num_nodes >= 0 && num_nodes < INT32_MAX, "block_plan_build: num_nodes out of range");
-    PTGNN_CHECK_ARG(T > 0 && T <= PTGNN_MAX_EDGE_TYPES && type_off, "block_plan_build: bad num_types=%d", T);
-    PTGNN_CHECK_ARG(B >= 8 && B <= 256, "block_plan_build: block_targets=%d must be in [8, 256]", B);
-    const int64_t E = type_off[T];
-    PTGNN_CHECK_ARG(E >= 0 && E < INT32_MAX, "block_plan_build: edge count out of range");
-    const int64_t nblk = ceil_div(num_nodes, B), groups = nblk * T;
-    PTGNN_CHECK_ARG(nblk * T * B < ((int64_t)1 << 31), "block_plan_build: %lld blocks x %d types x %d targets overflow the 31-bit sort key",
-                    (long long)nblk, T, B);
-    PTGNN_CHECK_ARG(group_off, "block_plan_build: null group_off");
-    const BlockPlanWs L = block_plan_ws_layout(num_nodes, E, T, B);
-    if (workspace_bytes < L.total || !workspace) {
-        set_error("block_plan_build: workspace %zu < required %zu", workspace_bytes, L.total);
-        return PTGNN_E_WORKSPACE;
-    }
-    PTGNN_CUDA(cudaMemsetAsync(group_off, 0, sizeof(int32_t) * (size_t)(groups + 1), st));
-    if (E == 0 || num_nodes == 0) return PTGNN_OK;
-    PTGNN_CHECK_ARG(src32 && tgt32 && src_f && tl_f, "block_plan_build: null edge array");
-    char *ws = static_cast<char *>(workspace);
-    int32_t *keys = reinterpret_cast<int32_t *>(ws + L.keys), *perm = reinterpret_cast<int32_t *>(ws + L.perm);
-    TypeOffsets toff{};
-    toff.num_types = T;
-    for (int t = 0; t <= PTGNN_MAX_EDGE_TYPES; ++t) toff.off[t] = (int32_t)type_off[t < T ? t : T];
-    const unsigned grid = (unsigned)(ceil_div(E, 256) < 132 * 16 ? ceil_div(E, 256) : 132 * 16);
-    {
-        TimedScope timed__(PTGNN_KERNEL_PLAN, st);
-        block_keys_kernel<<<grid, 256, 0, st>>>(toff, E, tgt32, B, keys, group_off);
-    }
-    PTGNN_LAUNCHED();
-    int rc = exclusive_scan_i32(group_off, group_off, groups + 1, reinterpret_cast<int32_t *>(ws + L.scan_sums), nullptr, st);
+    PTGNN_CHECK_ARG(num_types > 0 && num_types <= PTGNN_MAX_EDGE_TYPES && type_off, "block_plan_build: bad num_types=%d", num_types);
+    PlanJob J;
+    J.key = KEY_BLOCK;
+    J.N = J.N_src = num_nodes;
+    J.T = J.tabs.num_types = J.toff.num_types = num_types;
+    for (int t = 0; t <= PTGNN_MAX_EDGE_TYPES; ++t) {
+        J.tabs.off[t] = type_off[t < num_types ? t : num_types];
+        J.toff.off[t] = (int32_t)J.tabs.off[t];
+    }
+    J.E = type_off[num_types];
+    PTGNN_CHECK_ARG(J.E >= 0 && J.E < INT32_MAX, "block_plan_build: edge count out of range");
+    J.B = block_targets;
+    J.src32 = const_cast<int32_t *>(src32);
+    J.tgt32 = const_cast<int32_t *>(tgt32);
+    J.group_off = group_off; J.src_f = src_f; J.tl_f = tl_f;
+    int rc = check_block_args(J, "block_plan_build");
     if (rc) return rc;
-    const int32_t *sorted_keys = nullptr;
-    rc = sort_edges_by_key(keys, bits_for(nblk * T * B), E, perm, ws + L.plan, plan_ws_layout(num_nodes, E), st, &sorted_keys);
+    if (J.E > 0 && num_nodes > 0) PTGNN_CHECK_ARG(src32 && tgt32 && src_f && tl_f, "block_plan_build: null edge array");
+    return run_plan(J, workspace, workspace_bytes, static_cast<cudaStream_t>(stream));
+}
+
+extern "C" size_t ptgnn_b200_plan_convert_block_workspace_bytes(int64_t num_nodes, int64_t num_edges, int32_t num_types,
+                                                                int32_t block_targets) {
+    if (num_nodes < 0 || num_edges < 0 || num_types < 0 || block_targets <= 0) return 0;
+    const int64_t groups = ceil_div(num_nodes, block_targets) * num_types;
+    return plan_ws_layout(num_nodes, num_edges, true, groups, bits_for(groups * block_targets)).total;
+}
+
+extern "C" int ptgnn_b200_plan_convert_block(int64_t num_nodes, int64_t num_source_nodes, int32_t num_types,
+                                             const int64_t *const *src_ptrs, const int64_t *const *tgt_ptrs, const int64_t *counts,
+                                             int32_t block_targets, int32_t *row_ptr, int32_t *src32, int32_t *tgt32, int32_t *status,
+                                             int32_t *group_off, int32_t *src_f, uint8_t *tl_f, void *workspace, size_t workspace_bytes,
+                                             void *stream) {
+    PTGNN_CHECK_ARG(num_nodes >= 0 && num_nodes < INT32_MAX, "plan_convert_block: num_nodes=%lld out of range", (long long)num_nodes);
+    if (num_source_nodes <= 0) num_source_nodes = num_nodes;
+    PTGNN_CHECK_ARG(num_source_nodes < INT32_MAX, "plan_convert_block: num_source_nodes out of range");
+    PlanJob J;
+    int rc = job_edges(J, num_types, src_ptrs, tgt_ptrs, counts, true);
     if (rc) return rc;
-    {
-        TimedScope timed__(PTGNN_KERNEL_PLAN, st);
-        block_finalize_kernel<<<grid, 256, 0, st>>>(E, B, perm, sorted_keys, src32, src_f, tl_f);
-    }
-    PTGNN_LAUNCHED();
-    return PTGNN_OK;
-}
+    J.convert = true;
+    J.key = KEY_BLOCK;
+    J.N = num_nodes;
+    J.N_src = num_source_nodes;
+    J.B = block_targets;
+    J.src32 = src32; J.tgt32 = tgt32; J.row_ptr = row_ptr; J.status = status;
+    J.group_off = group_off; J.src_f = src_f; J.tl_f = tl_f;
+    rc = check_block_args(J, "plan_convert_block");
+    if (rc) return rc;
+    PTGNN_CHECK_ARG(row_ptr && status, "plan_convert_block: null row_ptr/status");
+    if (J.E > 0) {
+        PTGNN_CHECK_ARG(src32 && tgt32 && src_f && tl_f, "plan_convert_block: null output array");
+        PTGNN_CHECK_ARG(num_nodes > 0, "plan_convert_block: edges given but num_nodes == 0");
+    }
+    return run_plan(J, workspace, workspace_bytes, static_cast<cudaStream_t>(stream));
+}
diff --git a/ptgnn_b200/edgeplan.py b/ptgnn_b200/edgeplan.py
--- a/ptgnn_b200/edgeplan.py
+++ b/ptgnn_b200/edgeplan.py
@@ -13,8 +13,8 @@
 class EdgePlan:
 
     __slots__ = (
-        "num_nodes", "num_source_nodes", "num_edges", "num_types", "type_off", "type_off_c", "row_ptr", "src32", "tgt32", "status", "device", "_keepalive", "_validated", "_block", "_sorted", "_counts_c",
-        "_block_targets",
+        "num_nodes", "num_source_nodes", "num_edges", "num_types", "type_off", "type_off_c", "_row_ptr", "_src32", "_tgt32", "status", "device", "_keepalive", "_validated", "_block", "_sorted", "_counts_c",
+        "_block_targets", "_built",
     )
 
     STATUS_WORDS = 4
@@ -49,26 +49,51 @@
         def i32(n):
             return torch.empty(n, dtype=torch.int32, device=device)
 
-        self.row_ptr = i32(num_nodes + 1)
-        self.src32, self.tgt32 = i32(E), i32(E)
+        self._row_ptr = i32(num_nodes + 1)
+        self._src32, self._tgt32 = i32(E), i32(E)
         self._sorted = None
         self.status = torch.zeros(self.STATUS_WORDS, dtype=torch.int32).pin_memory()
         self._block = None
         self._counts_c = N.i64_array(counts)
-        lib = N.lib()
-        ws_bytes = lib.ptgnn_b200_plan_workspace_bytes(num_nodes, E)
-        ws = torch.empty(max(ws_bytes, 1), dtype=torch.uint8, device=device)
-        with torch.cuda.device(device):
-            rc = lib.ptgnn_b200_plan_convert(
-                num_nodes, self.num_source_nodes, len(counts), N.ptr_table(srcs), N.ptr_table(tgts), self._counts_c,
-                N.ptr(self.row_ptr), N.ptr(self.src32), N.ptr(self.tgt32), N.ptr(self.status), N.ptr(ws), ws_bytes,
-                N.current_stream(device),
-            )
-        N.check(rc, "ptgnn_b200_plan_convert")
         self._keepalive = (srcs, tgts)
+        self._built = False
         self._validated = False
         if validate:
             self.validate()
+
+    def _build(self, with_block_plan: bool = False) -> None:
+        if self._built:
+            return
+        srcs, tgts = self._keepalive
+        lib, dev, n, E = N.lib(), self.device, self.num_nodes, self.num_edges
+        common = (n, self.num_source_nodes, self.num_types, N.ptr_table(srcs), N.ptr_table(tgts), self._counts_c)
+        if with_block_plan:
+            B = self._resolve_block_targets()
+            group_off, src_f, tl_f = self._block_arrays(B)
+            ws_bytes = lib.ptgnn_b200_plan_convert_block_workspace_bytes(n, E, self.num_types, B)
+            ws = torch.empty(max(ws_bytes, 1), dtype=torch.uint8, device=dev)
+            with torch.cuda.device(dev):
+                rc = lib.ptgnn_b200_plan_convert_block(
+                    *common, B, N.ptr(self._row_ptr), N.ptr(self._src32), N.ptr(self._tgt32), N.ptr(self.status), N.ptr(group_off),
+                    N.ptr(src_f), N.ptr(tl_f), N.ptr(ws), ws_bytes, N.current_stream(dev))
+            N.check(rc, "ptgnn_b200_plan_convert_block")
+            self._set_block(B, group_off, src_f, tl_f)
+        else:
+            ws_bytes = lib.ptgnn_b200_plan_workspace_bytes(n, E)
+            ws = torch.empty(max(ws_bytes, 1), dtype=torch.uint8, device=dev)
+            with torch.cuda.device(dev):
+                rc = lib.ptgnn_b200_plan_convert(*common, N.ptr(self._row_ptr), N.ptr(self._src32), N.ptr(self._tgt32), N.ptr(self.status),
+                                                 N.ptr(ws), ws_bytes, N.current_stream(dev))
+            N.check(rc, "ptgnn_b200_plan_convert")
+        self._built = True
+
+    def _base(self):
+        self._build()
+        return self._row_ptr, self._src32, self._tgt32
+
+    row_ptr = property(lambda self: self._base()[0])
+    src32 = property(lambda self: self._base()[1])
+    tgt32 = property(lambda self: self._base()[2])
 
     def _sort(self):
         if self._sorted is None:
@@ -94,6 +119,7 @@
 
     def validate(self) -> None:
         if not self._validated:
+            self._build()
             torch.cuda.current_stream(self.device).synchronize()
             self.poll()
             self._validated = True
@@ -111,25 +137,37 @@
 
     def block_plan(self) -> "N.BlockPlanStruct":
         if self._block is None:
-            lib = N.lib()
-            B = self._block_targets
-            if B is None:
-                B = int(lib.ptgnn_b200_block_plan_block_targets(self.num_nodes))
-            nblk = (self.num_nodes + B - 1) // B
-            dev = self.device
-            group_off = torch.empty(nblk * self.num_types + 1, dtype=torch.int32, device=dev)
-            src_f = torch.empty(max(self.num_edges, 1), dtype=torch.int32, device=dev)
-            tl_f = torch.empty(max(self.num_edges, 1), dtype=torch.uint8, device=dev)
-            ws_bytes = lib.ptgnn_b200_block_plan_workspace_bytes(self.num_nodes, self.num_edges, self.num_types, B)
-            ws = torch.empty(max(ws_bytes, 1), dtype=torch.uint8, device=dev)
-            with torch.cuda.device(dev):
-                rc = lib.ptgnn_b200_block_plan_build(self.num_nodes, self.num_types, self.type_off_c, N.ptr(self.src32), N.ptr(self.tgt32),
-                                                     B, N.ptr(group_off), N.ptr(src_f), N.ptr(tl_f), N.ptr(ws), ws_bytes,
-                                                     N.current_stream(dev))
-            N.check(rc, "ptgnn_b200_block_plan_build")
-            struct = N.BlockPlanStruct(B, N.ptr(group_off), N.ptr(src_f), N.ptr(tl_f), self.status.data_ptr() + 4)
-            self._block = (struct, group_off, src_f, tl_f, B)
+            if not self._built:
+                self._build(with_block_plan=True)
+            else:
+                lib = N.lib()
+                B = self._resolve_block_targets()
+                group_off, src_f, tl_f = self._block_arrays(B)
+                dev = self.device
+                ws_bytes = lib.ptgnn_b200_block_plan_workspace_bytes(self.num_nodes, self.num_edges, self.num_types, B)
+                ws = torch.empty(max(ws_bytes, 1), dtype=torch.uint8, device=dev)
+                with torch.cuda.device(dev):
+                    rc = lib.ptgnn_b200_block_plan_build(self.num_nodes, self.num_types, self.type_off_c, N.ptr(self._src32),
+                                                         N.ptr(self._tgt32), B, N.ptr(group_off), N.ptr(src_f), N.ptr(tl_f), N.ptr(ws),
+                                                         ws_bytes, N.current_stream(dev))
+                N.check(rc, "ptgnn_b200_block_plan_build")
+                self._set_block(B, group_off, src_f, tl_f)
         return self._block[0]
+
+    def _resolve_block_targets(self) -> int:
+        B = self._block_targets
+        return int(N.lib().ptgnn_b200_block_plan_block_targets(self.num_nodes)) if B is None else B
+
+    def _block_arrays(self, B: int):
+        nblk = (self.num_nodes + B - 1) // B
+        dev = self.device
+        return (torch.empty(nblk * self.num_types + 1, dtype=torch.int32, device=dev),
+                torch.empty(max(self.num_edges, 1), dtype=torch.int32, device=dev),
+                torch.empty(max(self.num_edges, 1), dtype=torch.uint8, device=dev))
+
+    def _set_block(self, B: int, group_off, src_f, tl_f) -> None:
+        struct = N.BlockPlanStruct(B, N.ptr(group_off), N.ptr(src_f), N.ptr(tl_f), self.status.data_ptr() + 4)
+        self._block = (struct, group_off, src_f, tl_f, B)
 
     @property
     def block_targets(self) -> int:
```

After: 1.232 billion, median of 6. 1.5% higher.
